# edwinyosorahardjo/compressjs-flattened

Hardware: NVIDIA B200
Metric: bzip2-9 compress MB/s, byte-identical output (higher is better)
Workload: dtype u8

## Files before the change

### compressjs_flattened_b200/csrc/bwt.cuh

```cuda
#pragma once
#include "common.cuh"
#include "rle1.cuh"

#define SORT_TILE 4096
#ifndef SORT_THREADS
#define SORT_THREADS 512
#define SORT_E 8
#endif
#define SEG_THREADS 256
#define SEG_E 16
#define KEEP_BIT 0x80000000u

__global__ void __launch_bounds__(1024) k_tilemap(const u32 *__restrict__ seg_cnt, int nb, u32 *__restrict__ seg_tile0,
                                                  u32 *__restrict__ tile_blk, u64 *__restrict__ totals) {
  __shared__ u32 ws[33];
  __shared__ u64 ws64[33];
  u32 carry = 0;
  u64 act = 0;
  for (int base = 0; base < nb; base += blockDim.x) {
    int p = base + threadIdx.x;
    u32 c = p < nb ? seg_cnt[p] : 0;
    u32 tiles = (c + SORT_TILE - 1) / SORT_TILE, tot;
    u32 t0 = carry + block_excl_sum<u32>(tiles, tot, ws);
    if (p < nb) {
      seg_tile0[p] = t0;
      for (u32 t = 0; t < tiles; t++) tile_blk[t0 + t] = (u32)p;
    }
    carry += tot;
    act += block_sum<u64>((u64)c, ws64);
  }
  if (threadIdx.x == 0) { seg_tile0[nb] = carry; totals[0] = carry; totals[1] = act; }
}

__global__ void k_seg_init(const BlockRec *__restrict__ recs, int nb, u32 *__restrict__ seg_cnt) {
  int p = blockIdx.x * blockDim.x + threadIdx.x;
  if (p < nb) seg_cnt[p] = recs[p].n;
}

struct BlkSort {
  u32 cnt[256];
  u32 L, maxlen;
  u32 pad[6];
  u8 clen[256];
  u16 cval[256];
};
__global__ void __launch_bounds__(256) k_sym_used(const u8 *__restrict__ blk, i64 blk_stride, const BlockRec *__restrict__ recs,
                                                  BlkSort *__restrict__ bs) {
  __shared__ u32 h[8][256];
  const u32 p = blockIdx.y, n = recs[p].n;
  const u8 *T = blk + (i64)p * blk_stride;
  for (int i = threadIdx.x; i < 8 * 256; i += 256) (&h[0][0])[i] = 0;
  __syncthreads();
  u32 *hw = h[warp_id()];
  const u32 nv = n / 16;
  for (u32 x = blockIdx.x * 256 + threadIdx.x; x < nv; x += gridDim.x * 256) {
    uint4 v4 = reinterpret_cast<const uint4 *>(T)[x];
    u32 wv4[4] = {v4.x, v4.y, v4.z, v4.w};
#pragma unroll
    for (int k = 0; k < 16; k++) atomicAdd(&hw[(wv4[k >> 2] >> (8 * (k & 3))) & 0xffu], 1u);
  }
  if (blockIdx.x == 0)
    for (u32 i = nv * 16 + threadIdx.x; i < n; i += 256) atomicAdd(&hw[T[i]], 1u);
  __syncthreads();
  u32 tot = 0;
#pragma unroll
  for (int w = 0; w < 8; w++) tot += h[w][threadIdx.x];
  if (tot) atomicAdd(&bs[p].cnt[threadIdx.x], tot);
}
__global__ void __launch_bounds__(256) k_sym_tab(BlkSort *__restrict__ bs, u32 key_bits, u32 slack) {
  __shared__ u32 ws[33];
  __shared__ u32 P[257];
  __shared__ u32 wmax[8];
  BlkSort &B = bs[blockIdx.x];
  const u32 c = threadIdx.x;
  const u32 f = B.cnt[c];
  u32 used = f ? 1u : 0u, alpha;
  const u32 r = block_excl_sum<u32>(used, alpha, ws);
  u32 tot;
  const u32 pre = block_excl_sum<u32>(f, tot, ws);
  if (used) P[r] = pre;
  if (c == 0) P[alpha] = tot;
  __syncthreads();
  u32 len = 0, val = 0;
  if (used) {
    if (alpha == 1) { len = 1; val = 0; }
    else {
      u32 lb = 1;
      while ((1u << lb) < alpha) lb++;
      const u32 lmax = lb + (alpha > 2 ? slack : 0u);
      u32 lo = 0, hi = alpha;
      while (hi - lo > 1) {
        const u32 cap = 1u << (lmax - len - 1);
        const u64 mid2 = (u64)P[lo] + P[hi];
        u32 a = lo + 1, z = hi - 1;
        while (a < z) {
          const u32 m = (a + z) >> 1;
          if (2ull * P[m] < mid2) a = m + 1; else z = m;
        }
        u32 s = a;
        if (s > lo + 1 && 2ull * P[s] >= mid2 && mid2 - 2ull * P[s - 1] < 2ull * P[s] - mid2) s--;
        const u32 smin = hi > cap + lo ? hi - cap : lo + 1, smax = lo + cap < hi - 1 ? lo + cap : hi - 1;
        if (s < smin) s = smin;
        if (s > smax) s = smax;
        val <<= 1;
        if (r >= s) { val |= 1u; lo = s; } else hi = s;
        len++;
      }
    }
  }
  B.clen[c] = (u8)len;
  B.cval[c] = (u16)val;
  u32 mx = warp_max<u32>(len);
  if (lane_id() == 0) wmax[warp_id()] = mx;
  __syncthreads();
  if (c == 0) {
    u32 m = 1;
    for (int w = 0; w < 8; w++) if (wmax[w] > m) m = wmax[w];
    B.maxlen = m;
    B.L = key_bits / m;
  }
}
__global__ void __launch_bounds__(SEG_THREADS) k_keys_init(const u8 *__restrict__ blk, i64 blk_stride, const BlockRec *__restrict__ recs,
                                                           const u32 *__restrict__ seg_tile0, const u32 *__restrict__ tile_blk,
                                                           const BlkSort *__restrict__ bs, u64 *__restrict__ keys, u32 *__restrict__ hist0,
                                                           u32 tile_base, u32 key_bits) {
  __shared__ u32 cw[256];
  __shared__ u8 sc[SORT_TILE + 48];
  __shared__ u32 h[512];
  __shared__ u64 sk[SORT_TILE];
  u32 tile = blockIdx.x + tile_base, p = tile_blk[tile];
  u32 n = recs[p].n;
  cw[threadIdx.x] = ((u32)bs[p].clen[threadIdx.x] << 16) | bs[p].cval[threadIdx.x];
  for (int i = threadIdx.x; i < 512; i += SEG_THREADS) h[i] = 0;
  __syncthreads();
  const u8 *T = blk + (i64)p * blk_stride;
  u32 l0 = (tile - seg_tile0[p]) * SORT_TILE;
  u64 g0 = (u64)(tile - tile_base) * SORT_TILE;
  const u32 m = n - l0 < SORT_TILE ? n - l0 : SORT_TILE;
  for (u32 j = threadIdx.x; j < m + 43; j += SEG_THREADS) {
    u32 x = l0 + j;
    if (x >= n) x %= n;
    sc[j] = T[x];
  }
  __syncthreads();
  {
    const u32 j0 = threadIdx.x * SEG_E;
    u64 buf = 0;
    u32 bits = 0, kk = j0;
    for (u32 e = 0; e < SEG_E; e++) {
      const u32 j = j0 + e;
      if (j >= m) break;
      while (bits < key_bits) {
        const u32 w = cw[sc[kk++]], l = w >> 16;
        buf |= (u64)(w & 0xffffu) << (64 - bits - l);
        bits += l;
      }
      const u64 key = ((buf >> (64 - key_bits)) << 20) | (l0 + j);
      sk[j] = key;
      atomicAdd(&h[(u32)(key >> 20) & 511u], 1u);
      const u32 lj = cw[sc[j]] >> 16;
      buf <<= lj;
      bits -= lj;
    }
  }
  __syncthreads();
  for (u32 j = threadIdx.x; j < m; j += SEG_THREADS) keys[g0 + j] = sk[j];
  for (int i = threadIdx.x; i < 512; i += SEG_THREADS) hist0[(u64)(tile - tile_base) * 512 + i] = h[i];
}
template <int BITS>
__global__ void __launch_bounds__(SORT_THREADS) k_rs_hist(const u64 *__restrict__ keys, const u32 *__restrict__ seg_cnt,
                                                          const u32 *__restrict__ seg_tile0, const u32 *__restrict__ tile_blk, int shift,
                                                          u32 *__restrict__ hist, const u32 *__restrict__ seg_base, u32 tile_base = 0) {
  constexpr int NB = 1 << BITS;
  __shared__ u32 h[NB];
  u32 tile = blockIdx.x + tile_base, p = tile_blk[tile];
  u32 cnt = seg_cnt[p], l0 = (tile - seg_tile0[p]) * SORT_TILE;
  u64 g0 = seg_base ? (u64)seg_base[p] + l0 : (u64)(tile - tile_base) * SORT_TILE;
  for (int i = threadIdx.x; i < NB; i += SORT_THREADS) h[i] = 0;
  __syncthreads();
  u64 k[SORT_E];
#pragma unroll
  for (int e = 0; e < SORT_E; e++) {
    u32 o = e * SORT_THREADS + threadIdx.x;
    k[e] = l0 + o < cnt ? keys[g0 + o] : 0;
  }
#pragma unroll
  for (int e = 0; e < SORT_E; e++) {
    u32 o = e * SORT_THREADS + threadIdx.x;
    if (l0 + o < cnt) atomicAdd(&h[(u32)(k[e] >> shift) & (NB - 1)], 1u);
  }
  __syncthreads();
  for (int i = threadIdx.x; i < NB; i += SORT_THREADS) hist[(u64)(tile - tile_base) * NB + i] = h[i];
}
#define RSS_WARPS 16
template <int BITS>
__global__ void __launch_bounds__(RSS_WARPS * 32) k_rs_scan(u32 *__restrict__ hist, const u32 *__restrict__ seg_tile0, u32 *__restrict__ digit_tot,
                                                            u32 p_base = 0, u32 tile_base = 0) {
  constexpr int NB = 1 << BITS;
  __shared__ u32 part[RSS_WARPS][32];
  const u32 p = blockIdx.x + p_base, d = blockIdx.y * 32 + lane_id();
  const int w = warp_id();
  const u32 t0 = seg_tile0[p] - tile_base, t1 = seg_tile0[p + 1] - tile_base, nt = t1 - t0;
  const u32 per = (nt + RSS_WARPS - 1) / RSS_WARPS;
  const u32 a = t0 + (u32)w * per < t1 ? t0 + (u32)w * per : t1, b = a + per < t1 ? a + per : t1;
  u32 sum = 0;
  for (u32 t = a; t < b; t++) sum += hist[(u64)t * NB + d];
  part[w][lane_id()] = sum;
  __syncthreads();
  u32 acc = 0;
  for (int ww = 0; ww < w; ww++) acc += part[ww][lane_id()];
  if (w == RSS_WARPS - 1) digit_tot[(u64)p * NB + d] = acc + sum;
  for (u32 t = a; t < b; t++) {
    u32 v = hist[(u64)t * NB + d];
    hist[(u64)t * NB + d] = acc;
    acc += v;
  }
}
template <int BITS>
__global__ void __launch_bounds__(SORT_THREADS, 3) k_rs_scatter(const u64 *__restrict__ keys_in, u64 *__restrict__ keys_out,
                                                             const u32 *__restrict__ seg_cnt, const u32 *__restrict__ seg_tile0,
                                                             const u32 *__restrict__ tile_blk, int shift, const u32 *__restrict__ hist,
                                                             const u32 *__restrict__ digit_tot, const u32 *__restrict__ seg_base, u32 tile_base = 0) {
  constexpr int NB = 1 << BITS;
  __shared__ u16 wcnt[SORT_THREADS / 32][NB];
  __shared__ u32 base[NB];
  u32 tile = blockIdx.x + tile_base, p = tile_blk[tile];
  u32 cnt = seg_cnt[p], l0 = (tile - seg_tile0[p]) * SORT_TILE;
  u64 gp = seg_base ? (u64)seg_base[p] : (u64)(seg_tile0[p] - tile_base) * SORT_TILE, g0 = gp + l0;
  int lane = lane_id(), w = warp_id();
  for (int i = threadIdx.x; i < (SORT_THREADS / 32) * NB / 2; i += SORT_THREADS) reinterpret_cast<u32 *>(&wcnt[0][0])[i] = 0;
  {
    static_assert(NB <= SORT_THREADS, "one digit per thread");
    __shared__ u32 ws[33];
    u32 tot_d = threadIdx.x < NB ? digit_tot[(u64)p * NB + threadIdx.x] : 0u, tot;
    u32 ex = block_excl_sum<u32>(tot_d, tot, ws);
    if (threadIdx.x < NB) base[threadIdx.x] = ex + hist[(u64)(tile - tile_base) * NB + threadIdx.x];
  }
  __syncthreads();
  u64 key[SORT_E];
  u32 rk[SORT_E];
  u32 lt = (1u << lane) - 1;
#pragma unroll
  for (int e = 0; e < SORT_E; e++) {
    u32 o = (u32)w * (32 * SORT_E) + e * 32 + lane;
    key[e] = l0 + o < cnt ? keys_in[g0 + o] : 0;
  }
#pragma unroll
  for (int e = 0; e < SORT_E; e++) {
    u32 o = (u32)w * (32 * SORT_E) + e * 32 + lane;
    bool ok = l0 + o < cnt;
    u32 d = ok ? ((u32)(key[e] >> shift) & (NB - 1)) : (u32)NB;
    u32 peers = __match_any_sync(FULL_MASK, d);
    int leader = __ffs((int)peers) - 1;
    u32 old = 0;
    if (lane == leader && ok) { old = wcnt[w][d]; wcnt[w][d] = (u16)(old + __popc(peers)); }
    old = __shfl_sync(FULL_MASK, old, leader);
    rk[e] = old + __popc(peers & lt);
    __syncwarp();
  }
  __syncthreads();
  for (int d = threadIdx.x; d < NB; d += SORT_THREADS) {
    u32 acc = 0;
    for (int ww = 0; ww < SORT_THREADS / 32; ww++) { u32 t = wcnt[ww][d]; wcnt[ww][d] = (u16)acc; acc += t; }
  }
  __syncthreads();
#pragma unroll
  for (int e = 0; e < SORT_E; e++) {
    u32 o = (u32)w * (32 * SORT_E) + e * 32 + lane;
    if (l0 + o < cnt) {
      u32 d = (u32)(key[e] >> shift) & (NB - 1);
      u64 dst = gp + base[d] + wcnt[w][d] + rk[e];
      keys_out[dst] = key[e];
    }
  }
}

__device__ __forceinline__ void seg_load_flags(const u64 *__restrict__ keys, u64 g0, u32 l0, u32 cnt, int kshift, u64 k[SEG_E], u32 &flags, u32 &lbase) {
  lbase = l0 + threadIdx.x * SEG_E;
  u64 g = g0 + (u64)threadIdx.x * SEG_E;
  flags = 0;
  u64 prev = (lbase > 0 && lbase < cnt) ? keys[g - 1] : 0;
#pragma unroll
  for (int e = 0; e < SEG_E; e++) {
    if (lbase + e < cnt) {
      k[e] = keys[g + e];
      if (lbase + e == 0 || (k[e] >> kshift) != (prev >> kshift)) flags |= 1u << e;
      prev = k[e];
    }
  }
}
__global__ void __launch_bounds__(SEG_THREADS) k_sub_heads(const u64 *__restrict__ keys, const u32 *__restrict__ seg_cnt,
                                                           const u32 *__restrict__ seg_tile0, const u32 *__restrict__ tile_blk,
                                                           int *__restrict__ tile_last, const u32 *__restrict__ seg_base, int kshift) {
  __shared__ int ws[33];
  u32 tile = blockIdx.x, p = tile_blk[tile];
  u32 cnt = seg_cnt[p], l0 = (tile - seg_tile0[p]) * SORT_TILE;
  u64 k[SEG_E];
  u32 flags, lbase;
  seg_load_flags(keys, seg_base ? (u64)seg_base[p] + l0 : (u64)tile * SORT_TILE, l0, cnt, kshift, k, flags, lbase);
  int last = flags ? (int)(lbase + (31 - __clz((int)flags))) : -1;
  last = block_max<int>(last, ws);
  if (threadIdx.x == 0) tile_last[tile] = last;
}
__global__ void __launch_bounds__(256) k_seg_scan(const u32 *__restrict__ seg_tile0, int mode, const int *__restrict__ in, int *__restrict__ out,
                                                  u32 *__restrict__ seg_cnt_new) {
  __shared__ int ws[33];
  u32 p = blockIdx.x, t0 = seg_tile0[p], t1 = seg_tile0[p + 1];
  int carry = mode == 0 ? -1 : 0;
  for (u32 base = t0; base < t1; base += blockDim.x) {
    u32 t = base + threadIdx.x;
    int tot;
    if (mode == 0) {
      int v = t < t1 ? in[t] : -1;
      int e = block_excl_max<int>(v, -1, tot, ws);
      if (t < t1) out[t] = e > carry ? e : carry;
      if (tot > carry) carry = tot;
    } else {
      int v = t < t1 ? in[t] : 0;
      int e = block_excl_sum<int>(v, tot, ws);
      if (t < t1) out[t] = carry + e;
      carry += tot;
    }
  }
  if (mode == 1 && threadIdx.x == 0) seg_cnt_new[p] = (u32)carry;
}
__device__ __forceinline__ void bwt_emit_final(const u8 *__restrict__ T, u8 *__restrict__ L, BlockRec *__restrict__ recs, u32 p, u32 pb, u32 gidx,
                                               u32 rank) {
  if (gidx != pb) L[rank] = T[gidx - 1];
  else {
    L[rank] = T[pb + recs[p].n - 1];
    recs[p].orig_ptr = rank - pb;
  }
}

#define R0_THREADS 512
#define R0_ROWS (SORT_TILE / R0_THREADS)
#define R0_NOKEY 0xffffffffffffffffull
__global__ void __launch_bounds__(R0_THREADS) k_rank0(const u64 *__restrict__ keys, const u32 *__restrict__ seg_cnt,
                                                      const u32 *__restrict__ seg_tile0, const u32 *__restrict__ tile_blk,
                                                      u32 *__restrict__ isa, i64 stride, u32 *__restrict__ act_idx, u32 *__restrict__ act_rank,
                                                      u64 *__restrict__ status, u32 *__restrict__ ticket, u32 *__restrict__ n_act_out, u32 ntiles,
                                                      const u8 *__restrict__ T, u8 *__restrict__ L, BlockRec *__restrict__ recs, u32 tile_base) {
  __shared__ u64 sk[SORT_TILE + 2];
  __shared__ int wlast[R0_THREADS / 32];
  __shared__ u32 wkeep[R0_THREADS / 32];
  __shared__ u32 sh_tile, sh_base;
  __shared__ int sh_carry;
  const int lane = lane_id(), w = warp_id();
  if (threadIdx.x == 0) sh_tile = atomicAdd(ticket, 1u);
  __syncthreads();
  const u32 tile = sh_tile, p = tile_blk[tile];
  const u32 cnt = seg_cnt[p], l0 = (tile - seg_tile0[p]) * SORT_TILE;
  const u64 gp = (u64)(seg_tile0[p] - tile_base) * SORT_TILE;
  const u32 m = cnt - l0 < SORT_TILE ? cnt - l0 : SORT_TILE;
  for (u32 i = threadIdx.x; i < m + 2; i += R0_THREADS) {
    i64 j = (i64)l0 - 1 + i;
    sk[i] = (j >= 0 && j < (i64)cnt) ? keys[gp + (u64)j] : R0_NOKEY;
  }
  __syncthreads();
  u32 hb[R0_ROWS], kb[R0_ROWS];
  int wl = -1;
  u32 nkeep = 0;
#pragma unroll
  for (int e = 0; e < R0_ROWS; e++) {
    u32 i = (u32)w * (32 * R0_ROWS) + e * 32 + lane;
    bool valid = i < m, head = false, nh = false;
    if (valid) {
      u64 k = sk[i + 1] >> 20;
      head = l0 + i == 0 || k != (sk[i] >> 20);
      nh = l0 + i + 1 >= cnt || k != (sk[i + 2] >> 20);
    }
    hb[e] = __ballot_sync(FULL_MASK, head);
    kb[e] = __ballot_sync(FULL_MASK, valid && !(head && nh));
    if (hb[e]) wl = (int)(w * (32 * R0_ROWS) + e * 32 + (31 - __clz((int)hb[e])));
    nkeep += __popc(kb[e]);
  }
  if (lane == 0) { wlast[w] = wl; wkeep[w] = nkeep; }
  if (w == 0) {
    int carry = (int)l0;
    if (l0 > 0 && (sk[1] >> 20) == (sk[0] >> 20)) {
      const u64 P5 = sk[1] >> 20;
      const u64 *K = keys + gp;
      i64 res = -1;
      for (u32 c0 = 0; c0 < 64 && res < 0; c0 += 32) {
        i64 j = (i64)l0 - 2 - c0 - lane;
        bool diff = j < 0 || (K[j] >> 20) != P5;
        u32 b = __ballot_sync(FULL_MASK, diff);
        if (b) res = (i64)l0 - 1 - c0 - (__ffs((int)b) - 1);
      }
      if (res < 0) {
        u32 lo = 0, hi = l0 - 1;
        while (lo < hi) {
          u32 mid = (lo + hi) >> 1;
          if ((K[mid] >> 20) < P5) lo = mid + 1; else hi = mid;
        }
        res = lo;
      }
      carry = (int)res;
    }
    if (lane == 0) sh_carry = carry;
  }
  __syncthreads();
  int cur = sh_carry;
  for (int ww = 0; ww < w; ww++) if (wlast[ww] >= 0) cur = (int)l0 + wlast[ww];
  const u32 pb = (u32)((u64)p * (u64)stride);
  const u32 le = lane == 31 ? 0xffffffffu : ((2u << lane) - 1);
  const u32 lt = (1u << lane) - 1;
  u32 hpv[R0_ROWS];
#pragma unroll
  for (int e = 0; e < R0_ROWS; e++) {
    u32 i = (u32)w * (32 * R0_ROWS) + e * 32 + lane;
    u32 mk = hb[e] & le;
    int hp = mk ? (int)(l0 + w * (32 * R0_ROWS) + e * 32 + (31 - __clz((int)mk))) : cur;
    hpv[e] = (u32)hp;
    if (i < m) {
      const u32 gidx = pb + (u32)(sk[i + 1] & 0xFFFFFu);
      isa[gidx] = (u32)hp;
      if (!((kb[e] >> lane) & 1u)) bwt_emit_final(T, L, recs, p, pb, gidx, pb + (u32)hp);
    }
    if (hb[e]) cur = (int)(l0 + w * (32 * R0_ROWS) + e * 32 + (31 - __clz((int)hb[e])));
  }
  if (w == 0) {
    u32 x = lane < R0_THREADS / 32 ? wkeep[lane] : 0;
    u32 inc = warp_incl_sum<u32>(x);
    u32 agg = __shfl_sync(FULL_MASK, inc, 31);
    u32 base = lookback_warp(status, tile, agg);
    if (lane < R0_THREADS / 32) wkeep[lane] = inc - x;
    if (lane == 0) {
      sh_base = base;
      if (tile == ntiles - 1) *n_act_out = base + agg;
    }
  }
  __syncthreads();
  u32 out = sh_base + wkeep[w];
#pragma unroll
  for (int e = 0; e < R0_ROWS; e++) {
    u32 i = (u32)w * (32 * R0_ROWS) + e * 32 + lane;
    if (i < m && ((kb[e] >> lane) & 1u)) {
      u32 o = out + __popc(kb[e] & lt);
      act_idx[o] = pb + (u32)(sk[i + 1] & 0xFFFFFu);
      act_rank[o] = pb + hpv[e];
    }
    out += __popc(kb[e]);
  }
}
```

### compressjs_flattened_b200/csrc/bz2b200.cu

```cuda
#include "../../include/bz2b200.h"
#include "common.cuh"
#include "rle1.cuh"
#include "bwt.cuh"
#include "refine.cuh"
#include "rsort2.cuh"
#include "mtf.cuh"
#include "huff.cuh"
#include "decode.cuh"

#include <algorithm>
#include <atomic>
#include <chrono>
#include <condition_variable>
#include <future>
#include <mutex>
#include <thread>
#include <cctype>
#include <cstdio>
#include <cstdlib>
#include <fcntl.h>
#include <sched.h>
#include <sys/mman.h>
#include <sys/stat.h>
#include <unistd.h>
#include <string>
#include <utility>
#include <vector>

namespace {

struct ResultPool {
  std::mutex mu;
  std::vector<std::pair<void *, size_t>> live, idle;
  size_t idle_bytes = 0;
  static const size_t kMinPinned = 1 << 20, kMaxIdle = 48;
  static const size_t kMaxIdleBytes = (size_t)12 << 30;
  void *get(size_t bytes) {
    if (bytes < kMinPinned) return malloc(bytes ? bytes : 1);
    std::lock_guard<std::mutex> g(mu);
    size_t best = idle.size();
    for (size_t i = 0; i < idle.size(); i++)
      if (idle[i].second >= bytes && (best == idle.size() || idle[i].second < idle[best].second)) best = i;
    if (best < idle.size()) {
      auto e = idle[best];
      idle.erase(idle.begin() + (long)best);
      idle_bytes -= e.second;
      live.push_back(e);
      return e.first;
    }
    void *p = nullptr;
    size_t cap = bytes + bytes / 4 + 4096;
#ifndef BZ_SIM
    if (cudaMallocHost(&p, cap) != cudaSuccess) { cudaGetLastError(); p = nullptr; }
#endif
    if (!p) return malloc(bytes);
    live.push_back({p, cap});
    return p;
  }
  void put(void *p) {
    if (!p) return;
    {
      std::lock_guard<std::mutex> g(mu);
      for (size_t i = 0; i < live.size(); i++)
        if (live[i].first == p) {
          auto e = live[i];
          live.erase(live.begin() + (long)i);
          if (idle.size() < kMaxIdle && idle_bytes + e.second <= kMaxIdleBytes) { idle.push_back(e); idle_bytes += e.second; return; }
#ifndef BZ_SIM
          cudaFreeHost(p);
#endif
          return;
        }
    }
    free(p);
  }
};
ResultPool &result_pool() { static ResultPool rp; return rp; }

struct DevBuf {
  void *p = nullptr;
  size_t cap = 0;
};

struct Ctx;
struct Pool;
void pool_delete(Pool *p);
struct Ctx {
  Pool *own_pool = nullptr;
  size_t pool_min_bytes = 32000000;
  size_t pool_shard_bytes = 0, pool_halo0 = 0;
  bool pool_force_staging = false;
  int device = 0;
  cudaStream_t stream = nullptr;
  std::string err;
  bz2b200_stats st{};
  std::vector<DevBuf *> pool;
  DevBuf in, tile_last, tile_first, head_carry, tile_emit, g_sub, h_sub, g_tile, recs, nblk, blk, crcpart, pow256;
  DevBuf isa, keysA, keysB, valsB, actI0, actI1, actR0, actR1, lb_status, lbm, hist, digit_base;
  DevBuf seg_cnt, seg_tile0, tile_blk, tile_i0, tile_i1, totals;
  DevBuf Lcol, ranks, lastocc, A, freq, meta, W, bit_off, scrc, out, out_len, used_bits;
  DevBuf rs_tiles, gbounds;
  DevBuf key2, big_cnt, big_old, big_rank, big_tile0, big_tblk, totals2;
  DevBuf recs_cand, cand_first, out2, recs_all, blksort, r2_status, hfreq, hlens, hplen, hcodes, hsel, hcost, hgoff, hblk;
  DevBuf d_in, cand, ncand, dmeta, dsyms, dL, dtt, dwalk, dblk, dout, dmisc, dsel, doff, dperm, dmap;
  struct Pipe {
    const u8 *d_in = nullptr;
    i64 N = 0, T = 0, BS = 0, AS = 0, WS = 0;
    u32 B = 0;
    int level = 9, nb = 0;
    std::vector<BlockRec> hrecs;
  } pipe;
  bool trace = false;
  int sms = 148;
  unsigned ibwt_s = 64;
  u32 r0_tiles = 1u << 30;
  u32 key_slack = 2;
  u32 key_bits = 44;
  bool rs2 = false;
  int parse_mode = 0;
  std::vector<cudaEvent_t> trace_ev, trace_pool;
  std::vector<const char *> trace_names;
  void *rb_pin = nullptr;
  void *rb_dev = nullptr;
  const void *rb_src[4];
  void *rb_dst[4];
  size_t rb_off[4], rb_len[4], rb_used = 0;
  int rb_n = 0;
  u32 rb_seq = 0;
  bool ignore_block_crc = false;
  u32 cap_override = 0;
  u32 batch_override = 0;
  u32 dec_batch = 0;
  u64 shard_bits = 0;
  int cand_n = 0, cand_max_blocks = 0, cand_nb[64];
  i64 cand_s[64];
  bool recs_batched = false;
  int last_nb = 0;
  i64 last_bs = 0, last_as = 0;
  cudaEvent_t ev[10]{};
  bool ev_ok = false;
  std::vector<cudaEvent_t> dom_ev;
  size_t dom_used = 0;
  Ctx() {
    DevBuf *all[] = {&in, &tile_last, &tile_first, &head_carry, &tile_emit, &g_sub, &h_sub, &g_tile, &recs, &nblk, &blk, &crcpart, &pow256,
                     &isa, &keysA, &keysB, &valsB, &actI0, &actI1, &actR0, &actR1, &lb_status, &lbm, &hist, &digit_base,
                     &seg_cnt, &seg_tile0, &tile_blk, &tile_i0, &tile_i1, &totals,
                     &Lcol, &ranks, &lastocc, &A, &freq, &meta, &W, &bit_off, &scrc, &out, &out_len, &used_bits,
                     &rs_tiles, &gbounds, &key2, &big_cnt, &big_old, &big_rank, &big_tile0, &big_tblk, &totals2,
                     &recs_cand, &cand_first, &out2, &recs_all, &blksort, &r2_status, &hfreq, &hlens, &hplen, &hcodes, &hsel, &hcost, &hgoff, &hblk,
                     &d_in, &cand, &ncand, &dmeta, &dsyms, &dL, &dtt, &dwalk, &dblk, &dout, &dmisc, &dsel, &doff, &dperm, &dmap};
    for (DevBuf *b : all) pool.push_back(b);
  }
};

#define CK(call)                                                                         \
  do {                                                                                   \
    cudaError_t _e = (call);                                                             \
    if (_e != cudaSuccess) {                                                             \
      c->err = std::string(#call) + ": " + cudaGetErrorString(_e);                       \
      return BZ2B200_E_CUDA;                                                             \
    }                                                                                    \
  } while (0)

struct RbItem { const void *src; u32 off, bytes; };
__global__ void k_readback(RbItem i0, RbItem i1, RbItem i2, RbItem i3, int n, volatile u8 *host_page, u32 seq) {
  const RbItem it[4] = {i0, i1, i2, i3};
  for (int k = 0; k < n; k++)
    for (u32 b = threadIdx.x; b < it[k].bytes; b += blockDim.x) host_page[it[k].off + b] = reinterpret_cast<const u8 *>(it[k].src)[b];
  __threadfence_system();
  __syncthreads();
  if (threadIdx.x == 0) { *reinterpret_cast<volatile u32 *>(host_page + 1020) = seq; __threadfence_system(); }
}
int rb_add(Ctx *c, void *dst, const void *dev_src, size_t bytes) {
  if (!c->rb_pin) {
#ifndef BZ_SIM
    CK(cudaHostAlloc(&c->rb_pin, 1024, cudaHostAllocMapped));
    CK(cudaHostGetDevicePointer(&c->rb_dev, c->rb_pin, 0));
#else
    CK(cudaMallocHost(&c->rb_pin, 1024));
    c->rb_dev = c->rb_pin;
#endif
    memset(c->rb_pin, 0, 1024);
  }
  if (c->rb_n >= 4 || c->rb_used + bytes > 1000) { c->err = "internal: read-back scratch full"; return BZ2B200_E_CUDA; }
  c->rb_src[c->rb_n] = dev_src;
  c->rb_dst[c->rb_n] = dst; c->rb_off[c->rb_n] = c->rb_used; c->rb_len[c->rb_n] = bytes;
  c->rb_n++;
  c->rb_used += (bytes + 15) & ~(size_t)15;
  return 0;
}
int rb_sync(Ctx *c) {
  if (!c->rb_n) { CK(cudaStreamSynchronize(c->stream)); return 0; }
  RbItem it[4] = {};
  for (int i = 0; i < c->rb_n; i++) { it[i].src = c->rb_src[i]; it[i].off = (u32)c->rb_off[i]; it[i].bytes = (u32)c->rb_len[i]; }
  const u32 seq = ++c->rb_seq;
  KLAUNCH(k_readback, 1, 32, 0, c->stream, it[0], it[1], it[2], it[3], c->rb_n, (volatile u8 *)c->rb_dev, seq);
#ifndef BZ_SIM
  volatile u32 *flag = reinterpret_cast<volatile u32 *>((u8 *)c->rb_pin + 1020);
  for (unsigned spin = 0; *flag != seq; spin++) {
    if ((spin & 0xfffff) == 0xfffff && cudaStreamQuery(c->stream) != cudaErrorNotReady) {
      if (*flag == seq) break;
      CK(cudaStreamSynchronize(c->stream));
      CK(cudaGetLastError());
      c->err = "internal: read-back kernel did not publish";
      return BZ2B200_E_CUDA;
    }
  }
  std::atomic_thread_fence(std::memory_order_acquire);
#endif
  for (int i = 0; i < c->rb_n; i++) memcpy(c->rb_dst[i], (char *)c->rb_pin + c->rb_off[i], c->rb_len[i]);
  c->rb_n = 0;
  c->rb_used = 0;
  return 0;
}
#define RC(call)               \
  do {                         \
    int _r = (call);           \
    if (_r) return _r;         \
  } while (0)

void trace_mark(Ctx *c, const char *name, bool begin) {
#ifndef BZ_SIM
  cudaEvent_t e;
  if (c->trace_pool.size() > c->trace_ev.size()) e = c->trace_pool[c->trace_ev.size()];
  else { if (cudaEventCreate(&e) != cudaSuccess) return; c->trace_pool.push_back(e); }
  cudaEventRecord(e, c->stream);
  c->trace_ev.push_back(e);
  if (begin) c->trace_names.push_back(name);
#else
  (void)c; (void)name; (void)begin;
#endif
}
void trace_report(Ctx *c) {
#ifndef BZ_SIM
  if (!c->trace || c->trace_ev.empty()) return;
  cudaStreamSynchronize(c->stream);
  std::vector<std::pair<std::string, std::pair<int, float>>> agg;
  float gaps = 0, total = 0;
  for (size_t i = 0; i + 1 < c->trace_ev.size(); i += 2) {
    float ms = 0;
    cudaEventElapsedTime(&ms, c->trace_ev[i], c->trace_ev[i + 1]);
    const std::string nm = c->trace_names[i / 2];
    size_t k = 0;
    for (; k < agg.size(); k++) if (agg[k].first == nm) break;
    if (k == agg.size()) agg.push_back({nm, {0, 0.f}});
    agg[k].second.first++;
    agg[k].second.second += ms;
    total += ms;
    if (i + 2 < c->trace_ev.size()) { float g = 0; cudaEventElapsedTime(&g, c->trace_ev[i + 1], c->trace_ev[i + 2]); gaps += g; }
  }
  std::sort(agg.begin(), agg.end(), [](const auto &a, const auto &b) { return a.second.second > b.second.second; });
  fprintf(stderr, "[bz2b200 trace] %zu launches, kernels %.3f ms, gaps between launches %.3f ms\n", c->trace_names.size(), total, gaps);
  for (auto &a : agg) fprintf(stderr, "[bz2b200 trace] %-28s x%-3d %8.3f ms\n", a.first.c_str(), a.second.first, a.second.second);
  c->trace_ev.clear();
  c->trace_names.clear();
#else
  (void)c;
#endif
}

int ensure(Ctx *c, DevBuf &b, size_t bytes) {
  if (bytes <= b.cap) return 0;
  if (b.p) CK(cudaFree(b.p));
  b.p = nullptr;
  b.cap = 0;
  size_t want = bytes + bytes / 8 + 4096;
  CK(cudaMalloc(&b.p, want));
  b.cap = want;
  return 0;
}
#define ENS(buf, bytes)                         \
  do {                                          \
    int _r = ensure(c, (buf), (size_t)(bytes)); \
    if (_r) return _r;                          \
  } while (0)
template <typename T> T *P(DevBuf &b) { return reinterpret_cast<T *>(b.p); }

#define LAUNCH(kern, grid, block, smem, ...)                        \
  do {                                                              \
    if (c->trace) trace_mark(c, #kern, true);                       \
    KLAUNCH(kern, grid, block, smem, c->stream, __VA_ARGS__);       \
    if (c->trace) trace_mark(c, #kern, false);                      \
    c->st.kernel_launches++;                                        \
  } while (0)

inline i64 round_up(i64 v, i64 a) { return (v + a - 1) / a * a; }

int mark(Ctx *c, int i) {
  if (c->ev_ok) CK(cudaEventRecord(c->ev[i], c->stream));
  return 0;
}

int pipe_begin(Ctx *c, const u8 *d_in, size_t n_, int level) {
  if (level < 1 || level > 9) return BZ2B200_E_LEVEL;
  c->st = bz2b200_stats{};
  c->st.in_bytes = n_;
  c->err.clear();
  Ctx::Pipe &P_ = c->pipe;
  P_ = Ctx::Pipe{};
  P_.d_in = d_in; P_.N = (i64)n_; P_.level = level;
  P_.B = c->cap_override ? c->cap_override : (u32)level * 100000u - 19u;
  P_.T = (P_.N + RLE_TILE - 1) / RLE_TILE;
  const i64 N = P_.N, T = P_.T;
  int rc;
  if ((rc = mark(c, 0))) return rc;
  if (N > 0) {
    ENS(c->tile_last, 8 * T); ENS(c->tile_first, 8 * T); ENS(c->head_carry, 8 * T);
    ENS(c->tile_emit, 4 * T); ENS(c->g_tile, 8 * (T + 1));
    LAUNCH(k_rle_heads, (unsigned)T, RLE_THREADS, 0, d_in, N, P<i64>(c->tile_last), P<i64>(c->tile_first));
    LAUNCH(k_scan_excl_max_i64, 1, 1024, 0, P<i64>(c->tile_last), P<i64>(c->head_carry), T);
    ENS(c->g_sub, 4 * (size_t)T * (RLE_THREADS / 32)); ENS(c->h_sub, 8 * (size_t)T * (RLE_THREADS / 32));
    LAUNCH(k_rle_count, (unsigned)T, RLE_THREADS, 0, d_in, N, P<i64>(c->head_carry), P<u32>(c->tile_emit), P<u32>(c->g_sub), P<i64>(c->h_sub));
    LAUNCH(k_scan_excl_sum_u32_u64, 1, 1024, 0, P<u32>(c->tile_emit), P<u64>(c->g_tile), T);
  }
  return BZ2B200_OK;
}

#define CUT_CANDIDATES 64
int pipe_cut(Ctx *c, i64 s_start, i64 own_end, i64 g_start = -1) {
  Ctx::Pipe &P_ = c->pipe;
  const i64 N = P_.N, T = P_.T;
  const u32 B = P_.B;
  const int max_blocks = (int)(N / ((i64)B * 4 / 5) + 2);
  const int ncand = g_start >= 0 ? CUT_CANDIDATES : 1;
  ENS(c->recs, sizeof(BlockRec) * (size_t)max_blocks);
  ENS(c->nblk, 64 + 4 * CUT_CANDIDATES);
  int nb = 0;
  P_.hrecs.clear();
  c->cand_n = 0;
  if (N > 0 && g_start >= 0) {
    ENS(c->recs_cand, sizeof(BlockRec) * (size_t)max_blocks * ncand);
    LAUNCH(k_rle_cut, ncand, CUT_THREADS, 0, P_.d_in, N, B, P<u32>(c->g_sub), P<i64>(c->h_sub), P<i64>(c->tile_first), P<u64>(c->g_tile), T,
           P<BlockRec>(c->recs_cand), max_blocks, P<int>(c->nblk) + 16, s_start, own_end, g_start);
    LAUNCH(k_cand_firsts, 1, CUT_CANDIDATES, 0, P<BlockRec>(c->recs_cand), max_blocks, P<int>(c->nblk) + 16, P<i64>(c->cand_first));
    RC(rb_add(c, c->cand_nb, P<int>(c->nblk) + 16, 4 * CUT_CANDIDATES));
    RC(rb_add(c, c->cand_s, c->cand_first.p, 8 * CUT_CANDIDATES));
    RC(rb_sync(c));
    c->cand_n = ncand;
    c->cand_max_blocks = max_blocks;
  } else if (N > 0 && s_start < N && s_start < own_end) {
    LAUNCH(k_rle_cut, 1, CUT_THREADS, 0, P_.d_in, N, B, P<u32>(c->g_sub), P<i64>(c->h_sub), P<i64>(c->tile_first), P<u64>(c->g_tile), T,
           P<BlockRec>(c->recs), max_blocks, P<int>(c->nblk), s_start, own_end, (i64)-1);
    RC(rb_add(c, &nb, c->nblk.p, sizeof(int)));
    RC(rb_sync(c));
    if (nb < 0) { c->err = "internal: block table overflow"; return BZ2B200_E_CUDA; }
    P_.hrecs.resize((size_t)nb);
    if (nb) CK(cudaMemcpy(P_.hrecs.data(), c->recs.p, sizeof(BlockRec) * (size_t)nb, cudaMemcpyDeviceToHost));
  }
  P_.nb = nb;
  c->st.n_blocks = (u32)nb;
  return BZ2B200_OK;
}
bool pipe_pick(Ctx *c, i64 s_local, i64 own_end, int &rc) {
  Ctx::Pipe &P_ = c->pipe;
  rc = BZ2B200_OK;
  if (!(s_local < P_.N && s_local < own_end)) {
    P_.hrecs.clear();
    P_.nb = 0;
    c->st.n_blocks = 0;
    return true;
  }
  for (int j = 0; j < c->cand_n; j++) {
    const int nbj = c->cand_nb[j];
    if (nbj <= 0 || c->cand_s[j] != s_local) continue;
    P_.hrecs.resize((size_t)nbj);
    const BlockRec *src = P<BlockRec>(c->recs_cand) + (size_t)j * c->cand_max_blocks;
    if (cudaMemcpyAsync(c->recs.p, src, sizeof(BlockRec) * (size_t)nbj, cudaMemcpyDeviceToDevice, c->stream) != cudaSuccess ||
        cudaMemcpy(P_.hrecs.data(), src, sizeof(BlockRec) * (size_t)nbj, cudaMemcpyDeviceToHost) != cudaSuccess) { rc = BZ2B200_E_CUDA; return false; }
    P_.nb = nbj;
    c->st.n_blocks = (u32)nbj;
    return true;
  }
  return false;
}

int pipe_stages(Ctx *c) {
  Ctx::Pipe &P_ = c->pipe;
  const i64 N = P_.N, T = P_.T;
  const u32 B = P_.B;
  const int nb = P_.nb;
  const u8 *d_in = P_.d_in;
  std::vector<BlockRec> &hrecs = P_.hrecs;
  int rc;
  const i64 BS = round_up((i64)B + 1, 256);
  const i64 AS = round_up((i64)B + 2, 128);
  P_.BS = BS; P_.AS = AS;
  c->last_nb = nb; c->last_bs = BS; c->last_as = AS;
  ENS(c->meta, sizeof(BlockMeta) * (size_t)(nb + 1));
  ENS(c->bit_off, 8 * (size_t)(nb + 2));
  ENS(c->scrc, 64);
  ENS(c->out_len, 64);
  i64 WS = 0;
  if (nb) {
    ENS(c->blk, (size_t)nb * BS);
    const i64 t_first = hrecs.front().s / RLE_TILE, t_last = (hrecs.back().p + RLE_TILE - 1) / RLE_TILE;
    (void)T;
    LAUNCH(k_rle_emit, (unsigned)(t_last - t_first), RLE_THREADS, 0, d_in, N, B, P<i64>(c->head_carry), P<u64>(c->g_tile), P<BlockRec>(c->recs), nb,
           P<u8>(c->blk), BS, t_first);
    i64 max_len = 0;
    for (auto &r : hrecs) { if (r.p - r.s > max_len) max_len = r.p - r.s; c->st.rle1_bytes += r.n; }
    int max_chunks = (int)((max_len + CRC_CHUNK - 1) / CRC_CHUNK);
    ENS(c->crcpart, 4 * (size_t)nb * max_chunks);
    if (!c->pow256.p) {
      ENS(c->pow256, 1024);
      u32 h[256];
      for (int j = 0; j < 256; j++) h[j] = crc_xpow(8ull * 256 * (u64)j);
      CK(cudaMemcpy(c->pow256.p, h, sizeof h, cudaMemcpyHostToDevice));
    }
    LAUNCH(k_crc_chunks, dim3((unsigned)max_chunks, (unsigned)nb), 256, 0, d_in, P<BlockRec>(c->recs), P<u32>(c->pow256), P<u32>(c->crcpart),
           max_chunks);
    LAUNCH(k_crc_fold, (unsigned)((nb + 127) / 128), 128, 0, P<BlockRec>(c->recs), nb, P<u32>(c->crcpart), max_chunks,
           crc_xpow(8ull * CRC_CHUNK));
    if ((rc = mark(c, 1))) return rc;

    size_t slots = 0;
    std::vector<u32> tiles_of((size_t)nb), tile_first((size_t)nb);
    for (int b = 0; b < nb; b++) {
      tile_first[(size_t)b] = (u32)(slots / SORT_TILE);
      tiles_of[(size_t)b] = (u32)(round_up(hrecs[(size_t)b].n, SORT_TILE) / SORT_TILE);
      slots += (size_t)tiles_of[(size_t)b] * SORT_TILE;
    }
    const size_t tiles0 = slots / SORT_TILE;
    if ((u64)nb * (u64)BS >= (1ull << 31)) { c->err = "too many bytes for one call (block table * stride must stay below 2^31)"; return BZ2B200_E_ARG; }
    const size_t big_tiles = 5 * tiles0 + 16;
    const u32 big_cap = (u32)(slots / RF_T0 + 16);
    const size_t lb_tiles = slots / RF_T0 + tiles0 + 16;
    ENS(c->isa, 4 * (size_t)nb * BS);
    ENS(c->Lcol, (size_t)nb * BS);
    ENS(c->keysA, 8 * slots); ENS(c->keysB, 8 * slots);
    ENS(c->actI0, 4 * slots); ENS(c->actI1, 4 * slots); ENS(c->actR0, 4 * slots); ENS(c->actR1, 4 * slots);
    ENS(c->key2, 4 * slots);
    ENS(c->hist, 4 * 512 * big_tiles); ENS(c->digit_base, 4 * 512 * (size_t)(big_cap > (u32)nb ? big_cap : (u32)nb));
    ENS(c->seg_cnt, 4 * (size_t)nb); ENS(c->seg_tile0, 4 * (size_t)(nb + 1)); ENS(c->tile_blk, 4 * tiles0);
    ENS(c->tile_i0, 4 * big_tiles); ENS(c->tile_i1, 4 * big_tiles);
    ENS(c->big_cnt, 4 * (size_t)big_cap); ENS(c->big_old, 4 * (size_t)big_cap);
    ENS(c->big_rank, 4 * (size_t)big_cap); ENS(c->big_tile0, 4 * ((size_t)big_cap + 1)); ENS(c->big_tblk, 4 * big_tiles);
    ENS(c->lb_status, 8 * lb_tiles); ENS(c->lbm, 64);
    ENS(c->totals, 64); ENS(c->totals2, 64);
    u32 *seg_cnt = P<u32>(c->seg_cnt), *tile0 = P<u32>(c->seg_tile0), *tblk = P<u32>(c->tile_blk);
    u64 *kA = P<u64>(c->keysA), *kB = P<u64>(c->keysB);
    u32 *actI[2] = {P<u32>(c->actI0), P<u32>(c->actI1)}, *actR[2] = {P<u32>(c->actR0), P<u32>(c->actR1)};
    u32 *lbm = P<u32>(c->lbm);
    u64 *status = P<u64>(c->lb_status);
    const u64 magic = ~0ull / (u64)BS + 1;
    LAUNCH(k_seg_init, (unsigned)((nb + 255) / 256), 256, 0, P<BlockRec>(c->recs), nb, seg_cnt);
    LAUNCH(k_tilemap, 1, 1024, 0, seg_cnt, nb, tile0, tblk, P<u64>(c->totals));
    const unsigned Ta = (unsigned)tiles0;
    ENS(c->blksort, sizeof(BlkSort) * (size_t)nb);
    CK(cudaMemsetAsync(c->blksort.p, 0, sizeof(BlkSort) * (size_t)nb, c->stream));
    LAUNCH(k_sym_used, dim3(32, (unsigned)nb), 256, 0, P<u8>(c->blk), BS, P<BlockRec>(c->recs), P<BlkSort>(c->blksort));
    LAUNCH(k_sym_tab, (unsigned)nb, 256, 0, P<BlkSort>(c->blksort), c->key_bits, c->key_slack);
    ENS(c->rs_tiles, sizeof(RsTile) * (size_t)(Ta + 1));
    if (Ta) LAUNCH(k_rs_tiles, (Ta + 255) / 256, 256, 0, seg_cnt, tile0, tblk, (u32)Ta, P<RsTile>(c->rs_tiles));
    u64 total_n = 0;
    for (auto &r : hrecs) total_n += r.n;
    c->dom_used = 0;
    auto timed_scatter = [&](bool bits9, unsigned grid, const u64 *ki, u64 *ko, const u32 *scnt, const u32 *st0, const u32 *stb, int shift,
                             const u32 *sbase, u64 slots_now, u32 tile_base) -> int {
      if (c->ev_ok) {
        if (c->dom_used + 2 > c->dom_ev.size()) {
          cudaEvent_t a, b2;
          CK(cudaEventCreate(&a)); CK(cudaEventCreate(&b2));
          c->dom_ev.push_back(a); c->dom_ev.push_back(b2);
        }
        CK(cudaEventRecord(c->dom_ev[c->dom_used], c->stream));
      }
      if (bits9) LAUNCH(k_rs_scatter<9>, grid, SORT_THREADS, 0, ki, ko, scnt, st0, stb, shift, P<u32>(c->hist), P<u32>(c->digit_base), sbase, tile_base);
      else LAUNCH(k_rs_scatter<8>, grid, SORT_THREADS, 0, ki, ko, scnt, st0, stb, shift, P<u32>(c->hist), P<u32>(c->digit_base), sbase, tile_base);
      if (c->ev_ok) { CK(cudaEventRecord(c->dom_ev[c->dom_used + 1], c->stream)); c->dom_used += 2; }
      c->st.dom_launches++;
      c->st.dom_bytes += 16ull * slots_now;
      return 0;
    };
    u32 hv[4] = {0, 0, 0, 0};
    {
      c->st.sort_rounds++;
      c->st.sort_slots += (u64)Ta * SORT_TILE;
      CK(cudaMemsetAsync(lbm, 0, 16, c->stream));
      CK(cudaMemsetAsync(status, 0, 8 * (size_t)Ta, c->stream));
      for (int b0 = 0; b0 < nb;) {
        u32 gt = 0;
        int b1 = b0;
        u64 gn = 0;
        while (b1 < nb && (b1 == b0 || gt + tiles_of[b1] <= c->r0_tiles)) { gt += tiles_of[b1]; gn += hrecs[(size_t)b1].n; b1++; }
        const u32 tb = tile_first[b0];
        const unsigned gb = (unsigned)(b1 - b0);
        LAUNCH(k_keys_init, gt, SEG_THREADS, 0, P<u8>(c->blk), BS, P<BlockRec>(c->recs), tile0, tblk, P<BlkSort>(c->blksort), kA, P<u32>(c->hist), tb, c->key_bits);
        u64 *ki = kA, *ko = kB;
        const int npass = (int)(c->key_bits + 8) / 9;
        for (int pass = 0; pass < npass; pass++) {
          if (pass) LAUNCH(k_rs_hist<9>, gt, SORT_THREADS, 0, ki, seg_cnt, tile0, tblk, 20 + pass * 9, P<u32>(c->hist), (const u32 *)nullptr, tb);
          if (c->rs2 && tb == 0 && gt == Ta) {
#if RS2_SCAN1
            LAUNCH(k_rs_scan<9>, dim3((unsigned)nb, 512 / 32), RSS_WARPS * 32, 0, P<u32>(c->hist), tile0, P<u32>(c->digit_base), 0u, 0u);
#else
            LAUNCH(k_rs_bases, (unsigned)nb, 512, 0, P<u32>(c->hist), tile0);
#endif
            if (c->ev_ok) {
              if (c->dom_used + 2 > c->dom_ev.size()) {
                cudaEvent_t a, b2;
                CK(cudaEventCreate(&a)); CK(cudaEventCreate(&b2));
                c->dom_ev.push_back(a); c->dom_ev.push_back(b2);
              }
              CK(cudaEventRecord(c->dom_ev[c->dom_used], c->stream));
            }
            const unsigned g2 = gt < (unsigned)(2 * c->sms) ? gt : (unsigned)(2 * c->sms);
            LAUNCH(k_rs_scatter2, g2, RS2_THREADS, sizeof(Rs2Smem), ki, ko, P<u32>(c->hist), P<RsTile>(c->rs_tiles), gt, 20 + pass * 9, P<u32>(c->digit_base));
            if (c->ev_ok) { CK(cudaEventRecord(c->dom_ev[c->dom_used + 1], c->stream)); c->dom_used += 2; }
            c->st.dom_launches++;
            c->st.dom_bytes += 16ull * gn;
          } else {
            LAUNCH(k_rs_scan<9>, dim3(gb, 512 / 32), RSS_WARPS * 32, 0, P<u32>(c->hist), tile0, P<u32>(c->digit_base), (u32)b0, tb);
            if ((rc = timed_scatter(true, gt, ki, ko, seg_cnt, tile0, tblk, 20 + pass * 9, nullptr, gn, tb))) return rc;
          }
          u64 *tk = ki; ki = ko; ko = tk;
        }
        LAUNCH(k_rank0, gt, R0_THREADS, 0, ki, seg_cnt, tile0, tblk, P<u32>(c->isa), BS, actI[0], actR[0], status, lbm, lbm + 1, (u32)Ta, P<u8>(c->blk),
               P<u8>(c->Lcol), P<BlockRec>(c->recs), tb);
        b0 = b1;
      }
      RC(rb_add(c, hv, lbm, sizeof hv));
      RC(rb_sync(c));
    }
    u32 n_act = hv[1], round = 0;
    if (n_act) LAUNCH(k_keys2, (n_act + 255) / 256, 256, 0, actI[0], n_act, P<BlockRec>(c->recs), P<u32>(c->isa), (u32)BS, magic, P<BlkSort>(c->blksort), round,
                      P<u32>(c->key2));
    while (n_act) {
      c->st.sort_rounds++;
      c->st.sort_slots += n_act;
      const u32 ntiles = (n_act + RF_T0 - 1) / RF_T0, ctiles = (n_act + CK_TILE - 1) / CK_TILE;
      CK(cudaMemsetAsync(lbm, 0, 16, c->stream));
      CK(cudaMemsetAsync(status, 0, 8 * (size_t)ctiles, c->stream));
      ENS(c->gbounds, 8 * ((size_t)ntiles + 2));
      u32 *gb_lo = P<u32>(c->gbounds), *gb_lo2 = gb_lo + ntiles + 1;
      LAUNCH(k_group_bounds, (ntiles + 1 + 7) / 8, 256, 0, actR[0], n_act, ntiles, gb_lo, gb_lo2, P<u32>(c->big_cnt), P<u32>(c->big_old), P<u32>(c->big_rank),
             lbm + 2, big_cap);
      LAUNCH(k_sort_groups, ntiles, RF_THREADS, sizeof(RfSmem), P<u32>(c->key2), actI[0], actR[0], n_act, P<u32>(c->isa), (u32)BS, magic, actI[1],
             actR[1], P<u32>(c->big_cnt), P<u32>(c->big_old), P<u32>(c->big_rank), lbm + 2, big_cap, P<u8>(c->blk), P<u8>(c->Lcol), P<BlockRec>(c->recs),
             gb_lo, gb_lo2);
      RC(rb_add(c, hv, lbm, sizeof hv));
      RC(rb_sync(c));
      const u32 n_big = hv[2];
      if (n_big > big_cap) { c->err = "internal: big-group list overflow"; return BZ2B200_E_CUDA; }
      if (n_big) {
        u32 *bcnt = P<u32>(c->big_cnt), *bbase = P<u32>(c->big_old), *bt0 = P<u32>(c->big_tile0), *btb = P<u32>(c->big_tblk);
        u64 t2[2] = {0, 0};
        LAUNCH(k_tilemap, 1, 1024, 0, bcnt, (int)n_big, bt0, btb, P<u64>(c->totals2));
        RC(rb_add(c, t2, c->totals2.p, sizeof t2));
        RC(rb_sync(c));
        const unsigned Tb = (unsigned)t2[0];
        LAUNCH(k_big_keys, Tb, SEG_THREADS, 0, P<u32>(c->key2), actI[0], bcnt, bt0, btb, bbase, kA);
        u64 *ki = kA, *ko = kB;
        for (int pass = 0; pass < 3; pass++) {
          LAUNCH(k_rs_hist<8>, Tb, SORT_THREADS, 0, ki, bcnt, bt0, btb, 32 + pass * 8, P<u32>(c->hist), bbase);
          LAUNCH(k_rs_scan<8>, dim3(n_big, 256 / 32), RSS_WARPS * 32, 0, P<u32>(c->hist), bt0, P<u32>(c->digit_base));
          if ((rc = timed_scatter(false, Tb, ki, ko, bcnt, bt0, btb, 32 + pass * 8, bbase, t2[1], 0u))) return rc;
          u64 *tk = ki; ki = ko; ko = tk;
        }
        LAUNCH(k_sub_heads, Tb, SEG_THREADS, 0, ki, bcnt, bt0, btb, P<int>(c->tile_i0), bbase, 32);
        LAUNCH(k_seg_scan, n_big, 256, 0, bt0, 0, P<int>(c->tile_i0), P<int>(c->tile_i1), (u32 *)nullptr);
        LAUNCH(k_big_apply, Tb, SEG_THREADS, 0, ki, bcnt, bt0, btb, bbase, P<u32>(c->big_rank), P<int>(c->tile_i1), P<u32>(c->isa), (u32)BS, magic,
               actI[1], actR[1], P<u8>(c->blk), P<u8>(c->Lcol), P<BlockRec>(c->recs));
      }
      round = round < 30 ? round + 1 : round;
      LAUNCH(k_compact_keys, ctiles, CK_THREADS, 0, actI[1], actR[1], n_act, P<BlockRec>(c->recs), P<u32>(c->isa), (u32)BS, magic, P<BlkSort>(c->blksort), round,
             actI[0], actR[0],
             P<u32>(c->key2), status, lbm, lbm + 1, ctiles);
      RC(rb_add(c, hv, lbm, sizeof hv));
      RC(rb_sync(c));
      n_act = hv[1];
    }
    if ((rc = mark(c, 2))) return rc;

    const i64 nseg_max = (BS + MTF_SEG - 1) / MTF_SEG;
    ENS(c->ranks, (size_t)nb * BS);
    ENS(c->lastocc, 4 * 256 * (size_t)nseg_max * nb);
    ENS(c->A, 2 * (size_t)nb * AS);
    ENS(c->freq, 4 * BZ_MAX_SYMS * (size_t)nb);
    ENS(c->used_bits, 32 * (size_t)nb);
    CK(cudaMemsetAsync(c->used_bits.p, 0, 32 * (size_t)nb, c->stream));
    LAUNCH(k_mtf_lastocc, dim3((unsigned)((nseg_max + 7) / 8), (unsigned)nb), 256, 0, P<u8>(c->Lcol), BS, P<BlockRec>(c->recs), P<int>(c->lastocc),
           nseg_max * 256, P<u32>(c->used_bits));
    LAUNCH(k_mtf_scan, (unsigned)nb, 256, 0, P<BlockRec>(c->recs), P<int>(c->lastocc), nseg_max * 256, P<u32>(c->used_bits), P<BlockMeta>(c->meta));
    LAUNCH(k_mtf_ranks, dim3((unsigned)((nseg_max + MTR_WARPS - 1) / MTR_WARPS), (unsigned)nb), MTR_WARPS * 32, MTR_WARPS * sizeof(MtrSmem), P<u8>(c->Lcol),
           BS, P<BlockRec>(c->recs), P<int>(c->lastocc), nseg_max * 256, P<u8>(c->ranks));
    {
      const i64 r2_tiles = (BS + R2_TILE - 1) / R2_TILE;
      ENS(c->r2_status, 8 * (size_t)nb * r2_tiles + 4 * (size_t)nb);
      CK(cudaMemsetAsync(c->r2_status.p, 0, 8 * (size_t)nb * r2_tiles + 4 * (size_t)nb, c->stream));
      CK(cudaMemsetAsync(c->freq.p, 0, 4 * BZ_MAX_SYMS * (size_t)nb, c->stream));
      LAUNCH(k_mtf_rle2, dim3((unsigned)r2_tiles, (unsigned)nb), R2_THREADS, 0, P<BlockRec>(c->recs), P<u8>(c->ranks), BS, P<u16>(c->A), AS, P<u32>(c->freq),
             P<BlockMeta>(c->meta), P<u64>(c->r2_status), r2_tiles, reinterpret_cast<u32 *>(P<u64>(c->r2_status) + (size_t)nb * r2_tiles));
    }
    if ((rc = mark(c, 3))) return rc;

    u64 maxbits = 80 + 25 + 16 + 256 + 18 + 7ull * ((B + 1 + 49) / 50) + 6ull * (5 + 258 * 39) + 20ull * (B + 1);
    WS = round_up((i64)((maxbits + 31) / 32) + 2, 64);
    ENS(c->W, 4 * (size_t)nb * WS);
    const u32 max_nsel = (B + 1 + BZ_GROUP - 1) / BZ_GROUP;
    HufArrays ha;
    ha.sel_stride = round_up((i64)max_nsel + 1, 16);
    ENS(c->hfreq, 4 * (size_t)nb * BZ_MAX_GROUPS * BZ_MAX_SYMS);
    ENS(c->hlens, (size_t)nb * BZ_MAX_GROUPS * HUF_LSTRIDE);
    ENS(c->hplen, 8 * (size_t)nb * BZ_MAX_SYMS);
    ENS(c->hcodes, 4 * (size_t)nb * BZ_MAX_GROUPS * BZ_MAX_SYMS);
    ENS(c->hsel, (size_t)nb * ha.sel_stride);
    ENS(c->hcost, 2 * (size_t)nb * ha.sel_stride);
    ENS(c->hgoff, 4 * (size_t)nb * ha.sel_stride);
    ENS(c->hblk, sizeof(HufBlk) * (size_t)nb);
    ha.freq = P<u32>(c->hfreq); ha.lens = P<u8>(c->hlens); ha.plen = P<u64>(c->hplen); ha.codes = P<u32>(c->hcodes);
    ha.sel = P<u8>(c->hsel); ha.cost = P<u16>(c->hcost); ha.goff = P<u32>(c->hgoff); ha.hb = P<HufBlk>(c->hblk);
    const dim3 ggrid((max_nsel + HUF_GT - 1) / HUF_GT, (unsigned)nb);
    LAUNCH(k_huf_init, (unsigned)nb, HUF_BT, sizeof(HufBuildSmem), ha, P<u32>(c->freq), P<BlockMeta>(c->meta));
    for (int it = 0; it < BZ_MAX_GROUPS - 2; it++) {
      LAUNCH(k_huf_assign, ggrid, HUF_GT, 0, ha, P<u16>(c->A), AS, 0);
      LAUNCH(k_huf_split, (unsigned)nb, HUF_BT, 0, ha);
      LAUNCH(k_huf_hist, ggrid, HUF_GT, 0, ha, P<u16>(c->A), AS);
      LAUNCH(k_huf_build, (unsigned)nb, HUF_BT, sizeof(HufBuildSmem), ha);
    }
    LAUNCH(k_huf_assign, ggrid, HUF_GT, 0, ha, P<u16>(c->A), AS, 1);
    LAUNCH(k_huf_codes, (unsigned)nb, HUF_CT, 0, ha, P<BlockRec>(c->recs), P<BlockMeta>(c->meta), P<u32>(c->W), WS);
    LAUNCH(k_huf_emit, ggrid, HUF_GT, 0, ha, P<u16>(c->A), AS, P<u32>(c->W), WS);
  } else {
    for (int i = 1; i <= 3; i++) if ((rc = mark(c, i))) return rc;
  }
  P_.WS = WS;
  if ((rc = mark(c, 4))) return rc;
  return BZ2B200_OK;
}

int pipe_emit(Ctx *c, u64 base_bits, bool whole, u32 *d_out, size_t out_cap, bool own_out, size_t *out_len, u64 *bits_out, u32 *crc_fold) {
  Ctx::Pipe &P_ = c->pipe;
  const int nb = P_.nb;
  LAUNCH(k_stitch_offsets, 1, 1024, 0, P<BlockMeta>(c->meta), P<BlockRec>(c->recs), nb, P<u64>(c->bit_off), P<u32>(c->scrc), base_bits);
  u64 end_bits = 0;
  u32 fold = 0;
  RC(rb_add(c, &end_bits, P<u64>(c->bit_off) + nb, 8));
  RC(rb_add(c, &fold, c->scrc.p, 4));
  RC(rb_sync(c));
  if (bits_out) *bits_out = end_bits - base_bits;
  if (crc_fold) *crc_fold = fold;
  size_t need = (size_t)((end_bits + (whole ? 80 : 0) + 7) / 8);
  size_t need_w = round_up((i64)need, 4) + 8;
  if (own_out) {
    ENS(c->out, need_w);
    d_out = P<u32>(c->out);
  } else if (out_cap < need_w) {
    c->err = "output buffer too small";
    return BZ2B200_E_UNEXPECTED_OUTPUT_EOF;
  }
  CK(cudaMemsetAsync(d_out, 0, need_w, c->stream));
  if (nb) LAUNCH(k_stitch, dim3(32, (unsigned)nb), 256, 0, P<u32>(c->W), P_.WS, P<u64>(c->bit_off), d_out);
  u64 olen = need;
  if (whole) {
    LAUNCH(k_stream_ends, 1, 32, 0, d_out, P<u64>(c->bit_off), nb, P<u32>(c->scrc), P_.level, P<u64>(c->out_len));
    RC(rb_add(c, &olen, c->out_len.p, 8));
  }
  int rc;
  if ((rc = mark(c, 5))) return rc;
  RC(rb_sync(c));
  CK(cudaGetLastError());
  *out_len = (size_t)olen;
  c->st.out_bytes = olen;
  if (nb) {
    std::vector<BlockMeta> hm((size_t)nb);
    CK(cudaMemcpy(hm.data(), c->meta.p, sizeof(BlockMeta) * (size_t)nb, cudaMemcpyDeviceToHost));
    c->st.mtf_syms = 0;
    for (auto &m : hm) { c->st.mtf_syms += m.m; c->st.d1_triggered |= m.d1; }
  }
  if (c->ev_ok) {
    for (int i = 0; i < 5; i++) CK(cudaEventElapsedTime(&c->st.ms_stage[i], c->ev[i], c->ev[i + 1]));
    CK(cudaEventElapsedTime(&c->st.ms_total, c->ev[0], c->ev[5]));
    c->st.dom_ms = 0;
    for (size_t i = 0; i + 1 < c->dom_used; i += 2) {
      float ms = 0;
      CK(cudaEventElapsedTime(&ms, c->dom_ev[i], c->dom_ev[i + 1]));
      c->st.dom_ms += ms;
    }
  }
  return BZ2B200_OK;
}

int batch_limit(Ctx *c) {
  if (c->batch_override) return (int)c->batch_override;
  const i64 BS = round_up((i64)c->pipe.B + 1, 256);
  const i64 by_index = ((1ll << 31) - 1) / BS;
  i64 by_mem = by_index;
#ifndef BZ_SIM
  size_t pooled = 0;
  for (DevBuf *b : c->pool) pooled += b->cap;
  const size_t need = (size_t)c->pipe.nb * (size_t)BS * 52;
  if (need > pooled) {
    size_t free_b = 0, total_b = 0;
    if (cudaMemGetInfo(&free_b, &total_b) == cudaSuccess) by_mem = (i64)((free_b + pooled) / 10 * 7 / (size_t)(BS * 52));
  }
#endif
  i64 lim = by_index < by_mem ? by_index : by_mem;
  return (int)(lim < 1 ? 1 : lim);
}

int pipe_emit_part(Ctx *c, u64 base_bits, bool first, u32 *d_out, size_t out_cap, u64 *bits_out, u32 *crc_fold) {
  Ctx::Pipe &P_ = c->pipe;
  const int nb = P_.nb;
  LAUNCH(k_stitch_offsets, 1, 1024, 0, P<BlockMeta>(c->meta), P<BlockRec>(c->recs), nb, P<u64>(c->bit_off), P<u32>(c->scrc), base_bits);
  u64 end_bits = 0;
  u32 fold = 0;
  RC(rb_add(c, &end_bits, P<u64>(c->bit_off) + nb, 8));
  RC(rb_add(c, &fold, c->scrc.p, 4));
  RC(rb_sync(c));
  *bits_out = end_bits - base_bits;
  *crc_fold = fold;
  const u64 w_first = first ? 0 : (base_bits >> 5) + 1, w_end = ((end_bits + 80 + 31) >> 5) + 2;
  if (w_end * 4 > out_cap) { c->err = "output buffer too small"; return BZ2B200_E_UNEXPECTED_OUTPUT_EOF; }
  if (w_end > w_first) CK(cudaMemsetAsync(d_out + w_first, 0, (size_t)(w_end - w_first) * 4, c->stream));
  if (nb) LAUNCH(k_stitch, dim3(32, (unsigned)nb), 256, 0, P<u32>(c->W), P_.WS, P<u64>(c->bit_off), d_out);
  int rc;
  if ((rc = mark(c, 5))) return rc;
  CK(cudaStreamSynchronize(c->stream));
  CK(cudaGetLastError());
  return BZ2B200_OK;
}

int pipe_run(Ctx *c, u64 base_bits, bool whole, u32 *d_out, size_t out_cap, bool own_out, size_t *out_len, u64 *bits_out, u32 *crc_fold) {
  Ctx::Pipe &P_ = c->pipe;
  const int nb_total = P_.nb, maxb = batch_limit(c);
  int rc;
  c->recs_batched = false;
  if (nb_total <= maxb) {
    if ((rc = pipe_stages(c))) return rc;
    return pipe_emit(c, base_bits, whole, d_out, out_cap, own_out, out_len, bits_out, crc_fold);
  }
  std::vector<BlockRec> all = P_.hrecs;
  ENS(c->recs_all, sizeof(BlockRec) * (size_t)nb_total);
  CK(cudaMemcpyAsync(c->recs_all.p, c->recs.p, sizeof(BlockRec) * (size_t)nb_total, cudaMemcpyDeviceToDevice, c->stream));
  if (own_out) {
    out_cap = bz2b200_compress_bound((size_t)P_.N, P_.level) + 64;
    ENS(c->out, out_cap);
    d_out = P<u32>(c->out);
  }
  u64 running = base_bits, mtf_syms = 0;
  u32 fold = 0, d1 = 0;
  float ms_stage[5] = {0, 0, 0, 0, 0}, ms_total = 0, dom_ms = 0;
  for (int b0 = 0; b0 < nb_total; b0 += maxb) {
    const int bn = nb_total - b0 < maxb ? nb_total - b0 : maxb;
    CK(cudaMemcpyAsync(c->recs.p, P<BlockRec>(c->recs_all) + b0, sizeof(BlockRec) * (size_t)bn, cudaMemcpyDeviceToDevice, c->stream));
    P_.hrecs.assign(all.begin() + b0, all.begin() + b0 + bn);
    P_.nb = bn;
    if (b0) { if ((rc = mark(c, 0))) return rc; if ((rc = mark(c, 1))) return rc; }
    if ((rc = pipe_stages(c))) return rc;
    u64 bits = 0;
    u32 foldb = 0;
    if ((rc = pipe_emit_part(c, running, b0 == 0, d_out, out_cap, &bits, &foldb))) return rc;
    CK(cudaMemcpyAsync(P<BlockRec>(c->recs_all) + b0, c->recs.p, sizeof(BlockRec) * (size_t)bn, cudaMemcpyDeviceToDevice, c->stream));
    const u32 m = (u32)bn & 31u;
    fold = (m ? ((fold << m) | (fold >> (32 - m))) : fold) ^ foldb;
    running += bits;
    {
      std::vector<BlockMeta> hm((size_t)bn);
      CK(cudaMemcpy(hm.data(), c->meta.p, sizeof(BlockMeta) * (size_t)bn, cudaMemcpyDeviceToHost));
      for (auto &mm : hm) { mtf_syms += mm.m; d1 |= mm.d1; }
    }
    if (c->ev_ok) {
      for (int i = 0; i < 5; i++) { float t = 0; CK(cudaEventElapsedTime(&t, c->ev[i], c->ev[i + 1])); ms_stage[i] += t; ms_total += t; }
      for (size_t i = 0; i + 1 < c->dom_used; i += 2) { float t = 0; CK(cudaEventElapsedTime(&t, c->dom_ev[i], c->dom_ev[i + 1])); dom_ms += t; }
    }
  }
  P_.hrecs = all;
  P_.nb = nb_total;
  c->recs_batched = true;
  c->st.n_blocks = (u32)nb_total;
  if (bits_out) *bits_out = running - base_bits;
  if (crc_fold) *crc_fold = fold;
  u64 olen = (running + 7) / 8;
  if (whole) {
    u64 endb = running;
    CK(cudaMemcpyAsync(c->bit_off.p, &endb, 8, cudaMemcpyHostToDevice, c->stream));
    CK(cudaMemcpyAsync(c->scrc.p, &fold, 4, cudaMemcpyHostToDevice, c->stream));
    LAUNCH(k_stream_ends, 1, 32, 0, d_out, P<u64>(c->bit_off), 0, P<u32>(c->scrc), P_.level, P<u64>(c->out_len));
    RC(rb_add(c, &olen, c->out_len.p, 8));
    RC(rb_sync(c));
  }
  *out_len = (size_t)olen;
  c->st.out_bytes = olen;
  c->st.mtf_syms = mtf_syms;
  c->st.d1_triggered = d1;
  for (int i = 0; i < 5; i++) c->st.ms_stage[i] = ms_stage[i];
  c->st.ms_total = ms_total;
  c->st.dom_ms = dom_ms;
  return BZ2B200_OK;
}

int compress_device(Ctx *c, const u8 *d_in, size_t n_, int level, u32 *d_out, size_t out_cap, size_t *out_len, bool own_out) {
  int rc;
  if ((rc = pipe_begin(c, d_in, n_, level))) return rc;
  if ((rc = pipe_cut(c, 0, (i64)n_))) return rc;
  rc = pipe_run(c, 32, true, d_out, out_cap, own_out, out_len, nullptr, nullptr);
  trace_report(c);
  return rc;
}

#include "decode_host.inl"
#include "pool.inl"

cudaError_t set_kernel_attributes() {
#ifndef BZ_SIM
  cudaError_t e;
  if ((e = cudaFuncSetAttribute(k_sort_groups, cudaFuncAttributeMaxDynamicSharedMemorySize, (int)sizeof(RfSmem))) != cudaSuccess) return e;
  if ((e = cudaFuncSetAttribute(k_rs_scatter2, cudaFuncAttributeMaxDynamicSharedMemorySize, (int)sizeof(Rs2Smem))) != cudaSuccess) return e;
  if ((e = cudaFuncSetAttribute(k_mtf_ranks, cudaFuncAttributeMaxDynamicSharedMemorySize, (int)(MTR_WARPS * sizeof(MtrSmem)))) != cudaSuccess) return e;
  if ((e = cudaFuncSetAttribute(k_huf_init, cudaFuncAttributeMaxDynamicSharedMemorySize, (int)sizeof(HufBuildSmem))) != cudaSuccess) return e;
  if ((e = cudaFuncSetAttribute(k_huf_build, cudaFuncAttributeMaxDynamicSharedMemorySize, (int)sizeof(HufBuildSmem))) != cudaSuccess) return e;
  if ((e = cudaFuncSetAttribute(k_huff_parse_win, cudaFuncAttributeMaxDynamicSharedMemorySize, (int)sizeof(DecWinSmem))) != cudaSuccess) return e;
  const size_t rank_smem = 12 * (size_t)((DEC_DBUF_MAX + 64 - 1) / 64 + 2);
  if ((e = cudaFuncSetAttribute(k_ibwt_rank, cudaFuncAttributeMaxDynamicSharedMemorySize, (int)rank_smem)) != cudaSuccess) return e;
#endif
  return cudaSuccess;
}

int ctx_new(int device, Ctx **out) {
  int ndev = 0;
  if (cudaGetDeviceCount(&ndev) != cudaSuccess || ndev <= 0 || device < 0 || device >= ndev) return BZ2B200_E_CUDA;
  if (cudaSetDevice(device) != cudaSuccess) return BZ2B200_E_CUDA;
  Ctx *c = new Ctx();
  c->device = device;
  if (cudaStreamCreate(&c->stream) != cudaSuccess) { delete c; return BZ2B200_E_CUDA; }
  c->ev_ok = true;
  { const char *t = getenv("BZ2B200_TRACE"); c->trace = t && *t && *t != '0'; }
  { const char *t = getenv("BZ2B200_PARSE"); c->parse_mode = t ? atoi(t) : 0; }
  { const char *t = getenv("BZ2B200_KEY_SLACK"); if (t && *t >= '0' && *t <= '3') c->key_slack = (u32)(*t - '0'); }
  { const char *t = getenv("BZ2B200_KEY_BITS"); int v = t ? atoi(t) : 0; if (v == 36 || v == 44 || v == 27) c->key_bits = (u32)v; }
  { const char *t = getenv("BZ2B200_RS2"); if (t && *t) c->rs2 = *t != '0'; }
  { const char *t = getenv("BZ2B200_R0_TILES"); int v = t ? atoi(t) : 0; if (v > 0) c->r0_tiles = (u32)v; }
  { const char *t = getenv("BZ2B200_IBWT_S"); int v = t ? atoi(t) : 0; if (v == 64 || v == 128 || v == 256 || v == 512 || v == 1024) c->ibwt_s = (unsigned)v; }
  { int v = 0; if (cudaDeviceGetAttribute(&v, cudaDevAttrMultiProcessorCount, device) == cudaSuccess && v > 0) c->sms = v; }
  for (auto &e : c->ev) if (cudaEventCreate(&e) != cudaSuccess) c->ev_ok = false;
  if (set_kernel_attributes() != cudaSuccess) { ctx_delete(c); return BZ2B200_E_CUDA; }
  *out = c;
  return BZ2B200_OK;
}

void ctx_delete(Ctx *c) {
  if (!c) return;
  if (c->own_pool) pool_delete(c->own_pool);
  cudaSetDevice(c->device);
  for (DevBuf *b : c->pool) if (b->p) cudaFree(b->p);
  if (c->rb_pin) cudaFreeHost(c->rb_pin);
  for (auto &e : c->ev) if (e) cudaEventDestroy(e);
  for (auto &e : c->dom_ev) cudaEventDestroy(e);
  for (auto &e : c->trace_pool) cudaEventDestroy(e);
  cudaStreamDestroy(c->stream);
  delete c;
}

}

extern "C" {

int bz2b200_create(int device, bz2b200_ctx **ctx) {
  if (!ctx) return BZ2B200_E_ARG;
  *ctx = nullptr;
  Ctx *c = nullptr;
  int rc = ctx_new(device, &c);
  if (rc) return rc;
  *ctx = reinterpret_cast<bz2b200_ctx *>(c);
  return BZ2B200_OK;
}

void bz2b200_destroy(bz2b200_ctx *ctx) { ctx_delete(reinterpret_cast<Ctx *>(ctx)); }

int bz2b200_compress_device(bz2b200_ctx *ctx, const void *d_in, size_t n, int level, void *d_out, size_t out_cap, size_t *out_len) {
  Ctx *c = reinterpret_cast<Ctx *>(ctx);
  if (!c || !out_len || (n && !d_in) || !d_out || ((uintptr_t)d_in & 15) || ((uintptr_t)d_out & 3)) return BZ2B200_E_ARG;
  CK(cudaSetDevice(c->device));
  return compress_device(c, (const u8 *)d_in, n, level, (u32 *)d_out, out_cap, out_len, false);
}

int bz2b200_compress(bz2b200_ctx *ctx, const uint8_t *in, size_t n, int level, uint8_t **out, size_t *out_len) {
  Ctx *c = reinterpret_cast<Ctx *>(ctx);
  if (!c || !out || !out_len || (n && !in)) return BZ2B200_E_ARG;
  if (level < 1 || level > 9) return BZ2B200_E_LEVEL;
  CK(cudaSetDevice(c->device));
  if (n >= c->pool_min_bytes) {
    if (!c->own_pool) {
      const int dev = c->device;
      int prc = pool_new(&dev, 1, 2, &c->own_pool);
      if (prc) { c->err = "cannot create the lanes of the context's pool"; return prc; }
    }
    Pool *p = c->own_pool;
    p->cap_override = c->cap_override; p->batch_override = c->batch_override;
    p->halo0 = c->pool_halo0; p->force_staging = c->pool_force_staging;
    p->plan_first = n / 5 * 2 + 1;
    p->plan_growth = 1000.0;
    int prc = pool_compress_whole(p, in, n, level, c->pool_shard_bytes, out, out_len);
    c->st = p->st;
    c->err = p->err;
    return prc;
  }
  ENS(c->in, n + 64);
  if (n) CK(cudaMemcpyAsync(c->in.p, in, n, cudaMemcpyHostToDevice, c->stream));
  size_t olen = 0;
  int rc = compress_device(c, P<u8>(c->in), n, level, nullptr, 0, &olen, true);
  if (rc) return rc;
  uint8_t *res = (uint8_t *)result_pool().get(olen);
  if (!res) return BZ2B200_E_OUT_OF_MEMORY;
  CK(cudaMemcpy(res, c->out.p, olen, cudaMemcpyDeviceToHost));
  *out = res;
  *out_len = olen;
  return BZ2B200_OK;
}

int bz2b200_shard_begin(bz2b200_ctx *ctx, const void *in, size_t n_avail, int on_device, int level) {
  Ctx *c = reinterpret_cast<Ctx *>(ctx);
  if (!c || (n_avail && !in)) return BZ2B200_E_ARG;
  if (level < 1 || level > 9) return BZ2B200_E_LEVEL;
  CK(cudaSetDevice(c->device));
  const u8 *d_in = (const u8 *)in;
  if (!on_device) {
    ENS(c->in, n_avail + 64);
    if (n_avail) CK(cudaMemcpyAsync(c->in.p, in, n_avail, cudaMemcpyHostToDevice, c->stream));
    d_in = P<u8>(c->in);
  } else if ((uintptr_t)in & 15) return BZ2B200_E_ARG;
  return pipe_begin(c, d_in, n_avail, level);
}

static void shard_fill_info(Ctx *c, i64 s_start, int is_last, bz2b200_shard_info *info) {
  *info = bz2b200_shard_info{};
  const auto &h = c->pipe.hrecs;
  info->n_blocks = (uint32_t)h.size();
  info->next_start = h.empty() ? (uint64_t)(s_start < 0 ? 0 : s_start) : (uint64_t)h.back().p;
  info->complete = 1;
  if (!is_last && !h.empty() && h.back().p == c->pipe.N && h.back().n < c->pipe.B) info->complete = 0;
}

int bz2b200_shard_cut(bz2b200_ctx *ctx, uint64_t s_start, uint64_t own_len, int is_last, bz2b200_shard_info *info) {
  Ctx *c = reinterpret_cast<Ctx *>(ctx);
  if (!c || !info) return BZ2B200_E_ARG;
  CK(cudaSetDevice(c->device));
  if ((i64)own_len > c->pipe.N) own_len = (uint64_t)c->pipe.N;
  int rc = pipe_cut(c, (i64)s_start, (i64)own_len);
  if (rc) return rc;
  shard_fill_info(c, (i64)s_start, is_last, info);
  return BZ2B200_OK;
}

int bz2b200_shard_gtotal(bz2b200_ctx *ctx, uint64_t pos, uint64_t *g) {
  Ctx *c = reinterpret_cast<Ctx *>(ctx);
  if (!c || !g) return BZ2B200_E_ARG;
  CK(cudaSetDevice(c->device));
  const i64 N = c->pipe.N;
  *g = 0;
  if (N == 0) return BZ2B200_OK;
  ENS(c->nblk, 64 + 4 * CUT_CANDIDATES);
  LAUNCH(k_rle_gquery, 1, 32, 0, c->pipe.d_in, N, P<u32>(c->g_sub), P<i64>(c->h_sub), P<u64>(c->g_tile), c->pipe.T, (i64)(pos > (uint64_t)N ? (uint64_t)N : pos),
         P<u64>(c->nblk) + 1);
  u64 v = 0;
  RC(rb_add(c, &v, P<u64>(c->nblk) + 1, 8));
  RC(rb_sync(c));
  *g = v;
  return BZ2B200_OK;
}

int bz2b200_shard_cut_g(bz2b200_ctx *ctx, uint64_t g_before, uint64_t own_len) {
  Ctx *c = reinterpret_cast<Ctx *>(ctx);
  if (!c) return BZ2B200_E_ARG;
  CK(cudaSetDevice(c->device));
  c->cand_n = 0;
  if (c->pipe.N == 0) return BZ2B200_OK;
  if ((i64)own_len > c->pipe.N) own_len = (uint64_t)c->pipe.N;
  const u64 B = c->pipe.B, g_start = (B - g_before % B) % B;
  ENS(c->cand_first, 8 * CUT_CANDIDATES);
  return pipe_cut(c, 0, (i64)own_len, (i64)g_start);
}

int bz2b200_shard_cut_pick(bz2b200_ctx *ctx, uint64_t s_start, uint64_t own_len, int is_last, bz2b200_shard_info *info, int *found) {
  Ctx *c = reinterpret_cast<Ctx *>(ctx);
  if (!c || !info || !found) return BZ2B200_E_ARG;
  CK(cudaSetDevice(c->device));
  if ((i64)own_len > c->pipe.N) own_len = (uint64_t)c->pipe.N;
  int rc = BZ2B200_OK;
  *found = pipe_pick(c, (i64)s_start, (i64)own_len, rc) ? 1 : 0;
  if (rc) return rc;
  if (*found) shard_fill_info(c, (i64)s_start, is_last, info);
  return BZ2B200_OK;
}

int bz2b200_shard_compress(bz2b200_ctx *ctx, bz2b200_shard_info *info) {
  Ctx *c = reinterpret_cast<Ctx *>(ctx);
  if (!c || !info) return BZ2B200_E_ARG;
  CK(cudaSetDevice(c->device));
  size_t olen = 0;
  u64 bits = 0;
  u32 fold = 0;
  int rc = pipe_run(c, 0, false, nullptr, 0, true, &olen, &bits, &fold);
  if (rc) return rc;
  c->shard_bits = bits;
  info->bits = bits;
  info->crc_fold = fold;
  return BZ2B200_OK;
}

int bz2b200_shard_emit(bz2b200_ctx *ctx, int bit_phase, bz2b200_shard_info *info, uint8_t **seg, size_t *seg_bytes) {
  Ctx *c = reinterpret_cast<Ctx *>(ctx);
  if (!c || !info || !seg_bytes || bit_phase < 0 || bit_phase > 7) return BZ2B200_E_ARG;
  CK(cudaSetDevice(c->device));
  const u64 bits = c->shard_bits, nsrc = (bits + 7) / 8;
  const size_t olen = (size_t)(((u64)bit_phase + bits + 7) / 8);
  const u8 *d_seg = P<u8>(c->out);
  if (bit_phase && bits) {
    ENS(c->out2, nsrc + 16);
    LAUNCH(k_shift_bytes, (unsigned)((nsrc + 256) / 256), 256, 0, P<u8>(c->out), nsrc, (u32)bit_phase, P<u8>(c->out2));
    d_seg = P<u8>(c->out2);
  }
  CK(cudaStreamSynchronize(c->stream));
  info->bit_phase = (uint32_t)bit_phase;
  *seg_bytes = olen;
  if (!seg) return BZ2B200_OK;
  uint8_t *res = (uint8_t *)result_pool().get(olen);
  if (!res) return BZ2B200_E_OUT_OF_MEMORY;
  if (olen) CK(cudaMemcpy(res, d_seg, olen, cudaMemcpyDeviceToHost));
  *seg = res;
  *seg_bytes = olen;
  return BZ2B200_OK;
}

int bz2b200_stitch_shards(int level, int n_shards, const uint8_t *const *segs, const bz2b200_shard_info *infos, uint8_t **out, size_t *out_len) {
  if (level < 1 || level > 9) return BZ2B200_E_LEVEL;
  if (n_shards < 0 || !out || !out_len || (n_shards && (!segs || !infos))) return BZ2B200_E_ARG;
  u64 total_bits = 32;
  for (int r = 0; r < n_shards; r++) total_bits += infos[r].bits;
  size_t nbytes = (size_t)((total_bits + 80 + 7) / 8);
  uint8_t *o = (uint8_t *)calloc(nbytes + 8, 1);
  if (!o) return BZ2B200_E_OUT_OF_MEMORY;
  o[0] = 'B'; o[1] = 'Z'; o[2] = 'h'; o[3] = (uint8_t)('0' + level);
  u64 bitpos = 32;
  u32 crc = 0;
  for (int r = 0; r < n_shards; r++) {
    if (infos[r].bits) {
      if (infos[r].bit_phase != (u32)(bitpos & 7)) { free(o); return BZ2B200_E_ARG; }
      size_t off = (size_t)(bitpos >> 3), len = (size_t)((infos[r].bit_phase + infos[r].bits + 7) / 8);
      o[off] |= segs[r][0];
      if (len > 1) memcpy(o + off + 1, segs[r] + 1, len - 1);
      bitpos += infos[r].bits;
    }
    u32 m = infos[r].n_blocks & 31u;
    crc = (m ? ((crc << m) | (crc >> (32 - m))) : crc) ^ infos[r].crc_fold;
  }
  u64 vals[2] = {BZ_MAGIC_END, (u64)crc};
  int lens[2] = {48, 32};
  for (int q = 0; q < 2; q++)
    for (int i = lens[q] - 1; i >= 0; i--, bitpos++)
      if ((vals[q] >> i) & 1) o[bitpos >> 3] |= (uint8_t)(0x80u >> (bitpos & 7));
  *out = o;
  *out_len = (size_t)((bitpos + 7) / 8);
  return BZ2B200_OK;
}

size_t bz2b200_compress_bound(size_t n, int level) {
  if (level < 1 || level > 9) level = 9;
  size_t B = (size_t)level * 100000 - 19;
  size_t nblocks = n / (B * 4 / 5) + 2;
  return (n + n / 4 + nblocks) / 8 * 9 + nblocks * 22000 + 1024;
}

void bz2b200_free(void *p) { result_pool().put(p); }

const char *bz2b200_strerror(int rc) {
  switch (rc) {
    case BZ2B200_OK: return "OK";
    case BZ2B200_E_LAST_BLOCK: return "Bad file checksum";
    case BZ2B200_E_NOT_BZIP_DATA: return "Not bzip data";
    case BZ2B200_E_UNEXPECTED_INPUT_EOF: return "Unexpected input EOF";
    case BZ2B200_E_UNEXPECTED_OUTPUT_EOF: return "Unexpected output EOF";
    case BZ2B200_E_DATA_ERROR: return "Data error";
    case BZ2B200_E_OUT_OF_MEMORY: return "Out of memory";
    case BZ2B200_E_OBSOLETE_INPUT: return "Obsolete (pre 0.9.5) bzip format not supported.";
    case BZ2B200_E_LEVEL: return "Invalid block size multiplier";
    case BZ2B200_E_CUDA: return "CUDA failure";
    case BZ2B200_E_ARG: return "bad argument";
    case BZ2B200_E_PEER: return "a peer of the shard group failed or timed out";
    default: return "unknown error";
  }
}

const char *bz2b200_last_error(bz2b200_ctx *ctx) {
  Ctx *c = reinterpret_cast<Ctx *>(ctx);
  return c ? c->err.c_str() : "no context";
}

int bz2b200_last_stats(bz2b200_ctx *ctx, bz2b200_stats *st) {
  Ctx *c = reinterpret_cast<Ctx *>(ctx);
  if (!c || !st) return BZ2B200_E_ARG;
  *st = c->st;
  return BZ2B200_OK;
}

long long bz2b200_debug_fetch(bz2b200_ctx *ctx, int what, int blk, void *dst, size_t cap) {
  Ctx *c = reinterpret_cast<Ctx *>(ctx);
  if (!c || !dst) return BZ2B200_E_ARG;
  const void *src = nullptr;
  size_t bytes = 0;
  int nb = c->last_nb;
  if (what != 0 && what != 4 && (blk < 0 || blk >= nb)) return BZ2B200_E_ARG;
  switch (what) {
    case 0:
      if (c->recs_batched) { src = c->recs_all.p; bytes = sizeof(BlockRec) * (size_t)c->pipe.nb; }
      else { src = c->recs.p; bytes = sizeof(BlockRec) * (size_t)nb; }
      break;
    case 1: src = P<u8>(c->blk) + (i64)blk * c->last_bs; bytes = (size_t)c->last_bs; break;
    case 2: src = P<u8>(c->Lcol) + (i64)blk * c->last_bs; bytes = (size_t)c->last_bs; break;
    case 3: src = P<u16>(c->A) + (i64)blk * c->last_as; bytes = 2 * (size_t)c->last_as; break;
    case 4: src = c->meta.p; bytes = sizeof(BlockMeta) * (size_t)nb; break;
    default: return BZ2B200_E_ARG;
  }
  if (bytes > cap) bytes = cap;
  if (bytes && cudaMemcpy(dst, src, bytes, cudaMemcpyDeviceToHost) != cudaSuccess) return BZ2B200_E_CUDA;
  return (long long)bytes;
}

int bz2b200_debug_huffman_lengths(bz2b200_ctx *ctx, int32_t *a, int n, int maxlen) {
  Ctx *c = reinterpret_cast<Ctx *>(ctx);
  if (!c || !a || n < 0 || n > 1 << 20 || maxlen < 1 || maxlen > 32) return BZ2B200_E_ARG;
  CK(cudaSetDevice(c->device));
  if (!n) return BZ2B200_OK;
  ENS(c->dmisc, 4 * (size_t)n + 64);
  CK(cudaMemcpyAsync(c->dmisc.p, a, 4 * (size_t)n, cudaMemcpyHostToDevice, c->stream));
  LAUNCH(k_debug_ha_allocate, 1, 32, 0, P<int>(c->dmisc), n, maxlen);
  CK(cudaMemcpyAsync(a, c->dmisc.p, 4 * (size_t)n, cudaMemcpyDeviceToHost, c->stream));
  CK(cudaStreamSynchronize(c->stream));
  return BZ2B200_OK;
}

int bz2b200_debug_set_batch_blocks(bz2b200_ctx *ctx, uint32_t blocks) {
  Ctx *c = reinterpret_cast<Ctx *>(ctx);
  if (!c) return BZ2B200_E_ARG;
  c->batch_override = blocks;
  return BZ2B200_OK;
}

int bz2b200_debug_set_ignore_block_crc(bz2b200_ctx *ctx, int on) {
  Ctx *c = reinterpret_cast<Ctx *>(ctx);
  if (!c) return BZ2B200_E_ARG;
  c->ignore_block_crc = on != 0;
  return BZ2B200_OK;
}

int bz2b200_debug_set_block_cap(bz2b200_ctx *ctx, uint32_t cap) {
  Ctx *c = reinterpret_cast<Ctx *>(ctx);
  if (!c || (cap && cap < 8) || cap > 899981) return BZ2B200_E_ARG;
  c->cap_override = cap;
  return BZ2B200_OK;
}

#include "decode_abi.inl"
#include "pool_abi.inl"
#include "stream_abi.inl"

}
```

### compressjs_flattened_b200/csrc/rsort2.cuh

```cuda
#pragma once
#include "common.cuh"
#include "bwt.cuh"

struct RsTile {
  u32 p;
  u32 m;
  u32 g0;
  u32 gp;
};
__global__ void k_rs_tiles(const u32 *__restrict__ seg_cnt, const u32 *__restrict__ seg_tile0, const u32 *__restrict__ tile_blk, u32 ntiles,
                           RsTile *__restrict__ info) {
  u32 t = blockIdx.x * blockDim.x + threadIdx.x;
  if (t >= ntiles) return;
  u32 p = tile_blk[t], l0 = (t - seg_tile0[p]) * SORT_TILE, cnt = seg_cnt[p];
  RsTile r;
  r.p = p; r.m = cnt - l0 < SORT_TILE ? cnt - l0 : SORT_TILE; r.g0 = t * SORT_TILE; r.gp = seg_tile0[p] * SORT_TILE;
  info[t] = r;
}

__global__ void __launch_bounds__(512) k_rs_bases(u32 *__restrict__ hist, const u32 *__restrict__ seg_tile0) {
  __shared__ u32 ws[33];
  const u32 p = blockIdx.x, d = threadIdx.x;
  const u32 t0 = seg_tile0[p], t1 = seg_tile0[p + 1];
  u32 sum = 0;
  for (u32 t = t0; t < t1; t++) sum += hist[(u64)t * 512 + d];
  u32 tot;
  u32 acc = block_excl_sum<u32>(sum, tot, ws);
  for (u32 t = t0; t < t1; t++) {
    const u32 v = hist[(u64)t * 512 + d];
    hist[(u64)t * 512 + d] = acc;
    acc += v;
  }
}

#ifndef RS2_BALLOT
#define RS2_BALLOT 0
#endif
#ifndef RS2_PACK
#define RS2_PACK 1
#endif
#ifndef RS2_SCAN1
#define RS2_SCAN1 1
#endif
#ifndef RS2_DIRECT
#define RS2_DIRECT 0
#endif
#define RS2_THREADS 512
#define RS2_WARPS (RS2_THREADS / 32)
struct Rs2Smem {
  u64 keys[2][SORT_TILE];
  u32 gbase[2][512];
#if RS2_SCAN1
  u32 dtot[2][512];
#endif
#if RS2_PACK
  u32 wcnt[RS2_WARPS / 2][512];
#else
  u32 wcnt[RS2_WARPS][512];
#endif
  u32 lpos[512];
  u32 delta[512];
  u32 ws[34];
  u64 ws64[34];
  RsTile info[2];
  u64 mbar[2];
};

#ifndef BZ_SIM
__device__ __forceinline__ u32 smem_u32(const void *p) { return (u32)__cvta_generic_to_shared(p); }
__device__ __forceinline__ void mbar_init(u64 *bar, u32 count) { asm volatile("mbarrier.init.shared::cta.b64 [%0], %1;" ::"r"(smem_u32(bar)), "r"(count)); }
__device__ __forceinline__ void mbar_expect_tx(u64 *bar, u32 bytes) {
  asm volatile("mbarrier.arrive.expect_tx.shared::cta.b64 _, [%0], %1;" ::"r"(smem_u32(bar)), "r"(bytes) : "memory");
}
__device__ __forceinline__ void tma_load_1d(void *dst, const void *src, u32 bytes, u64 *bar) {
  asm volatile("cp.async.bulk.shared::cluster.global.mbarrier::complete_tx::bytes [%0], [%1], %2, [%3];" ::"r"(smem_u32(dst)), "l"(src), "r"(bytes),
               "r"(smem_u32(bar))
               : "memory");
}
__device__ __forceinline__ void mbar_wait(u64 *bar, u32 parity) {
  asm volatile(
      "{\n"
      ".reg .pred p;\n"
      "RS2_WAIT:\n"
      "mbarrier.try_wait.parity.shared::cta.b64 p, [%0], %1;\n"
      "@p bra RS2_DONE;\n"
      "bra RS2_WAIT;\n"
      "RS2_DONE:\n"
      "}\n" ::"r"(smem_u32(bar)),
      "r"(parity)
      : "memory");
}
#endif

__device__ __forceinline__ void rs2_fetch(Rs2Smem &sm, int b, u32 tile, const u64 *__restrict__ keys_in, const u32 *__restrict__ hist,
                                          const RsTile *__restrict__ tinfo, const u32 *__restrict__ digit_tot) {
  const RsTile ti = tinfo[tile];
  sm.info[b] = ti;
  const u32 kbytes = ((ti.m * 8u) + 15u) & ~15u;
#ifndef BZ_SIM
  asm volatile("fence.proxy.async.shared::cta;" ::: "memory");
  mbar_expect_tx(&sm.mbar[b], kbytes + 2048u * (1 + RS2_SCAN1));
  tma_load_1d(sm.keys[b], keys_in + ti.g0, kbytes, &sm.mbar[b]);
  tma_load_1d(sm.gbase[b], hist + (u64)tile * 512, 2048u, &sm.mbar[b]);
#if RS2_SCAN1
  tma_load_1d(sm.dtot[b], digit_tot + (u64)ti.p * 512, 2048u, &sm.mbar[b]);
#endif
#else
  for (u32 i = 0; i < kbytes / 8; i++) sm.keys[b][i] = keys_in[ti.g0 + i];
  for (u32 i = 0; i < 512; i++) sm.gbase[b][i] = hist[(u64)tile * 512 + i];
#if RS2_SCAN1
  for (u32 i = 0; i < 512; i++) sm.dtot[b][i] = digit_tot[(u64)ti.p * 512 + i];
#endif
#endif
  (void)digit_tot;
}

__global__ void __launch_bounds__(RS2_THREADS, 2) k_rs_scatter2(const u64 *__restrict__ keys_in, u64 *__restrict__ keys_out, const u32 *__restrict__ hist,
                                                                const RsTile *__restrict__ tinfo, u32 ntiles, int shift,
                                                                const u32 *__restrict__ digit_tot) {
  DYN_SMEM(Rs2Smem, smp);
  Rs2Smem &sm = *smp;
  const int lane = lane_id(), w = warp_id();
  const u32 lt = (1u << lane) - 1;
  if (threadIdx.x == 0) {
#ifndef BZ_SIM
    mbar_init(&sm.mbar[0], 1);
    mbar_init(&sm.mbar[1], 1);
    asm volatile("fence.mbarrier_init.release.cluster;" ::: "memory");
#endif
  }
  __syncthreads();
  u32 tile = blockIdx.x;
  if (threadIdx.x == 0 && tile < ntiles) rs2_fetch(sm, 0, tile, keys_in, hist, tinfo, digit_tot);
  for (u32 it = 0; tile < ntiles; it++, tile += gridDim.x) {
    const int b = (int)(it & 1);
    if (threadIdx.x == 0 && tile + gridDim.x < ntiles) rs2_fetch(sm, b ^ 1, tile + gridDim.x, keys_in, hist, tinfo, digit_tot);
#ifndef BZ_SIM
    mbar_wait(&sm.mbar[b], (it >> 1) & 1u);
#else
    __syncthreads();
#endif
    const u32 m = sm.info[b].m, gp = sm.info[b].gp;
    u64 key[SORT_E];
    u32 rk[SORT_E];
#pragma unroll
    for (int e = 0; e < SORT_E; e++) {
      const u32 o = (u32)w * (32 * SORT_E) + e * 32 + lane;
      key[e] = o < m ? sm.keys[b][o] : 0;
    }
#if RS2_PACK
    for (int i = threadIdx.x; i < RS2_WARPS / 2 * 512; i += RS2_THREADS) (&sm.wcnt[0][0])[i] = 0;
#else
    for (int i = threadIdx.x; i < RS2_WARPS * 512; i += RS2_THREADS) (&sm.wcnt[0][0])[i] = 0;
#endif
    u32 dg[SORT_E], peers[SORT_E];
#pragma unroll
    for (int e = 0; e < SORT_E; e++) {
      const u32 o = (u32)w * (32 * SORT_E) + e * 32 + lane;
      dg[e] = o < m ? ((u32)(key[e] >> shift) & 511u) : 512u;
#if RS2_BALLOT
      u32 pm = __ballot_sync(FULL_MASK, o < m);
      if (!(o < m)) pm = ~pm;
#pragma unroll
      for (int bit = 0; bit < 9; bit++) {
        const bool one = (dg[e] >> bit) & 1u;
        const u32 bal = __ballot_sync(FULL_MASK, one);
        pm &= one ? bal : ~bal;
      }
      peers[e] = pm;
#else
      peers[e] = __match_any_sync(FULL_MASK, dg[e]);
#endif
    }
    __syncthreads();
#pragma unroll
    for (int e = 0; e < SORT_E; e++) {
      const int leader = __ffs((int)peers[e]) - 1;
      u32 old = 0;
#if RS2_PACK
      if (lane == leader && dg[e] < 512u) old = (atomicAdd(&sm.wcnt[w >> 1][dg[e]], (u32)__popc(peers[e]) << (16 * (w & 1))) >> (16 * (w & 1))) & 0xffffu;
#else
      if (lane == leader && dg[e] < 512u) old = atomicAdd(&sm.wcnt[w][dg[e]], (u32)__popc(peers[e]));
#endif
      old = __shfl_sync(FULL_MASK, old, leader);
      rk[e] = old + __popc(peers[e] & lt);
    }
    __syncthreads();
    {
      const u32 d = threadIdx.x;
      u32 acc = 0;
#if RS2_PACK
      u32 cw[RS2_WARPS / 2];
#pragma unroll
      for (int q = 0; q < RS2_WARPS / 2; q++) {
        const u32 v = sm.wcnt[q][d], lo = v & 0xffffu, hi = v >> 16;
        cw[q] = acc | ((acc + lo) << 16);
        acc += lo + hi;
      }
#if RS2_SCAN1
      u64 tot64;
      const u64 ex = block_excl_sum<u64>(((u64)sm.dtot[b][d] << 32) | acc, tot64, reinterpret_cast<u64 *>(sm.ws64));
      const u32 lp = (u32)ex, dbase = (u32)(ex >> 32);
#else
      u32 tot;
      const u32 lp = block_excl_sum<u32>(acc, tot, sm.ws);
      const u32 dbase = 0;
#endif
#pragma unroll
      for (int q = 0; q < RS2_WARPS / 2; q++) sm.wcnt[q][d] = cw[q] + lp * 0x10001u;
#else
      u32 cw[RS2_WARPS];
#pragma unroll
      for (int ww = 0; ww < RS2_WARPS; ww++) { cw[ww] = acc; acc += sm.wcnt[ww][d]; }
      u32 tot;
      const u32 lp = block_excl_sum<u32>(acc, tot, sm.ws);
      const u32 dbase = 0;
#pragma unroll
      for (int ww = 0; ww < RS2_WARPS; ww++) sm.wcnt[ww][d] = lp + cw[ww];
#endif
      sm.lpos[d] = lp;
      sm.delta[d] = dbase + sm.gbase[b][d] - lp;
    }
    __syncthreads();
#if RS2_DIRECT
#pragma unroll
    for (int e = 0; e < SORT_E; e++)
      if (dg[e] < 512u) {
#if RS2_PACK
        const u32 slot = ((sm.wcnt[w >> 1][dg[e]] >> (16 * (w & 1))) & 0xffffu) + rk[e];
#else
        const u32 slot = sm.wcnt[w][dg[e]] + rk[e];
#endif
        keys_out[(u64)gp + sm.delta[dg[e]] + slot] = key[e];
      }
#else
#pragma unroll
    for (int e = 0; e < SORT_E; e++)
      if (dg[e] < 512u) {
#if RS2_PACK
        sm.keys[b][((sm.wcnt[w >> 1][dg[e]] >> (16 * (w & 1))) & 0xffffu) + rk[e]] = key[e];
#else
        sm.keys[b][sm.wcnt[w][dg[e]] + rk[e]] = key[e];
#endif
      }
    __syncthreads();
    for (u32 i = threadIdx.x; i < m; i += RS2_THREADS) {
      const u64 k = sm.keys[b][i];
      keys_out[(u64)gp + sm.delta[(u32)(k >> shift) & 511u] + i] = k;
    }
#endif
    __syncthreads();
  }
}
```

Baseline: 7449.

## Replace tiled radix passes with per-bucket merge sort for small digit buckets

Removes the TMA-pipelined rs_scatter2 path and the tile_base chunking. It adds a planning kernel that groups small digit buckets (at most 4096 keys) into work items and finishes each item with a shared-memory bitonic-network-plus-merge-path sort. Only oversized buckets are forwarded to further radix passes. The aim is to skip full-array radix passes for keys already separated by the top digit, at the cost of device atomics for item allocation and padded shared-memory merge passes.

```diff
diff --git a/compressjs_flattened_b200/csrc/bwt.cuh b/compressjs_flattened_b200/csrc/bwt.cuh
--- a/compressjs_flattened_b200/csrc/bwt.cuh
+++ b/compressjs_flattened_b200/csrc/bwt.cuh
@@ -12,9 +12,10 @@
 #define KEEP_BIT 0x80000000u
 
 __global__ void __launch_bounds__(1024) k_tilemap(const u32 *__restrict__ seg_cnt, int nb, u32 *__restrict__ seg_tile0,
-                                                  u32 *__restrict__ tile_blk, u64 *__restrict__ totals) {
+                                                  u32 *__restrict__ tile_blk, u64 *__restrict__ totals, const u32 *__restrict__ nb_dev = nullptr) {
   __shared__ u32 ws[33];
   __shared__ u64 ws64[33];
+  if (nb_dev) nb = (int)*nb_dev;
   u32 carry = 0;
   u64 act = 0;
   for (int base = 0; base < nb; base += blockDim.x) {
@@ -123,19 +124,19 @@
 __global__ void __launch_bounds__(SEG_THREADS) k_keys_init(const u8 *__restrict__ blk, i64 blk_stride, const BlockRec *__restrict__ recs,
                                                            const u32 *__restrict__ seg_tile0, const u32 *__restrict__ tile_blk,
                                                            const BlkSort *__restrict__ bs, u64 *__restrict__ keys, u32 *__restrict__ hist0,
-                                                           u32 tile_base, u32 key_bits) {
+                                                           u32 hshift, u32 key_bits) {
   __shared__ u32 cw[256];
   __shared__ u8 sc[SORT_TILE + 48];
   __shared__ u32 h[512];
   __shared__ u64 sk[SORT_TILE];
-  u32 tile = blockIdx.x + tile_base, p = tile_blk[tile];
+  u32 tile = blockIdx.x, p = tile_blk[tile];
   u32 n = recs[p].n;
   cw[threadIdx.x] = ((u32)bs[p].clen[threadIdx.x] << 16) | bs[p].cval[threadIdx.x];
   for (int i = threadIdx.x; i < 512; i += SEG_THREADS) h[i] = 0;
   __syncthreads();
   const u8 *T = blk + (i64)p * blk_stride;
   u32 l0 = (tile - seg_tile0[p]) * SORT_TILE;
-  u64 g0 = (u64)(tile - tile_base) * SORT_TILE;
+  u64 g0 = (u64)tile * SORT_TILE;
   const u32 m = n - l0 < SORT_TILE ? n - l0 : SORT_TILE;
   for (u32 j = threadIdx.x; j < m + 43; j += SEG_THREADS) {
     u32 x = l0 + j;
@@ -157,7 +158,7 @@
       }
       const u64 key = ((buf >> (64 - key_bits)) << 20) | (l0 + j);
       sk[j] = key;
-      atomicAdd(&h[(u32)(key >> 20) & 511u], 1u);
+      atomicAdd(&h[(u32)(key >> hshift) & 511u], 1u);
       const u32 lj = cw[sc[j]] >> 16;
       buf <<= lj;
       bits -= lj;
@@ -165,17 +166,17 @@
   }
   __syncthreads();
   for (u32 j = threadIdx.x; j < m; j += SEG_THREADS) keys[g0 + j] = sk[j];
-  for (int i = threadIdx.x; i < 512; i += SEG_THREADS) hist0[(u64)(tile - tile_base) * 512 + i] = h[i];
+  for (int i = threadIdx.x; i < 512; i += SEG_THREADS) hist0[(u64)tile * 512 + i] = h[i];
 }
 template <int BITS>
 __global__ void __launch_bounds__(SORT_THREADS) k_rs_hist(const u64 *__restrict__ keys, const u32 *__restrict__ seg_cnt,
                                                           const u32 *__restrict__ seg_tile0, const u32 *__restrict__ tile_blk, int shift,
-                                                          u32 *__restrict__ hist, const u32 *__restrict__ seg_base, u32 tile_base = 0) {
+                                                          u32 *__restrict__ hist, const u32 *__restrict__ seg_base) {
   constexpr int NB = 1 << BITS;
   __shared__ u32 h[NB];
-  u32 tile = blockIdx.x + tile_base, p = tile_blk[tile];
+  u32 tile = blockIdx.x, p = tile_blk[tile];
   u32 cnt = seg_cnt[p], l0 = (tile - seg_tile0[p]) * SORT_TILE;
-  u64 g0 = seg_base ? (u64)seg_base[p] + l0 : (u64)(tile - tile_base) * SORT_TILE;
+  u64 g0 = seg_base ? (u64)seg_base[p] + l0 : (u64)tile * SORT_TILE;
   for (int i = threadIdx.x; i < NB; i += SORT_THREADS) h[i] = 0;
   __syncthreads();
   u64 k[SORT_E];
@@ -190,17 +191,16 @@
     if (l0 + o < cnt) atomicAdd(&h[(u32)(k[e] >> shift) & (NB - 1)], 1u);
   }
   __syncthreads();
-  for (int i = threadIdx.x; i < NB; i += SORT_THREADS) hist[(u64)(tile - tile_base) * NB + i] = h[i];
+  for (int i = threadIdx.x; i < NB; i += SORT_THREADS) hist[(u64)tile * NB + i] = h[i];
 }
 #define RSS_WARPS 16
 template <int BITS>
-__global__ void __launch_bounds__(RSS_WARPS * 32) k_rs_scan(u32 *__restrict__ hist, const u32 *__restrict__ seg_tile0, u32 *__restrict__ digit_tot,
-                                                            u32 p_base = 0, u32 tile_base = 0) {
+__global__ void __launch_bounds__(RSS_WARPS * 32) k_rs_scan(u32 *__restrict__ hist, const u32 *__restrict__ seg_tile0, u32 *__restrict__ digit_tot) {
   constexpr int NB = 1 << BITS;
   __shared__ u32 part[RSS_WARPS][32];
-  const u32 p = blockIdx.x + p_base, d = blockIdx.y * 32 + lane_id();
+  const u32 p = blockIdx.x, d = blockIdx.y * 32 + lane_id();
   const int w = warp_id();
-  const u32 t0 = seg_tile0[p] - tile_base, t1 = seg_tile0[p + 1] - tile_base, nt = t1 - t0;
+  const u32 t0 = seg_tile0[p], t1 = seg_tile0[p + 1], nt = t1 - t0;
   const u32 per = (nt + RSS_WARPS - 1) / RSS_WARPS;
   const u32 a = t0 + (u32)w * per < t1 ? t0 + (u32)w * per : t1, b = a + per < t1 ? a + per : t1;
   u32 sum = 0;
@@ -220,13 +220,13 @@
 __global__ void __launch_bounds__(SORT_THREADS, 3) k_rs_scatter(const u64 *__restrict__ keys_in, u64 *__restrict__ keys_out,
                                                              const u32 *__restrict__ seg_cnt, const u32 *__restrict__ seg_tile0,
                                                              const u32 *__restrict__ tile_blk, int shift, const u32 *__restrict__ hist,
-                                                             const u32 *__restrict__ digit_tot, const u32 *__restrict__ seg_base, u32 tile_base = 0) {
+                                                             const u32 *__restrict__ digit_tot, const u32 *__restrict__ seg_base) {
   constexpr int NB = 1 << BITS;
   __shared__ u16 wcnt[SORT_THREADS / 32][NB];
   __shared__ u32 base[NB];
-  u32 tile = blockIdx.x + tile_base, p = tile_blk[tile];
+  u32 tile = blockIdx.x, p = tile_blk[tile];
   u32 cnt = seg_cnt[p], l0 = (tile - seg_tile0[p]) * SORT_TILE;
-  u64 gp = seg_base ? (u64)seg_base[p] : (u64)(seg_tile0[p] - tile_base) * SORT_TILE, g0 = gp + l0;
+  u64 gp = seg_base ? (u64)seg_base[p] : (u64)seg_tile0[p] * SORT_TILE, g0 = gp + l0;
   int lane = lane_id(), w = warp_id();
   for (int i = threadIdx.x; i < (SORT_THREADS / 32) * NB / 2; i += SORT_THREADS) reinterpret_cast<u32 *>(&wcnt[0][0])[i] = 0;
   {
@@ -234,7 +234,7 @@
     __shared__ u32 ws[33];
     u32 tot_d = threadIdx.x < NB ? digit_tot[(u64)p * NB + threadIdx.x] : 0u, tot;
     u32 ex = block_excl_sum<u32>(tot_d, tot, ws);
-    if (threadIdx.x < NB) base[threadIdx.x] = ex + hist[(u64)(tile - tile_base) * NB + threadIdx.x];
+    if (threadIdx.x < NB) base[threadIdx.x] = ex + hist[(u64)tile * NB + threadIdx.x];
   }
   __syncthreads();
   u64 key[SORT_E];
@@ -273,6 +273,100 @@
       keys_out[dst] = key[e];
     }
   }
+}
+
+#define R0_CAP 4096
+#define R0_ITEM_OTHER (1ull << 63)
+#define R0_PLAN_THREADS 128
+__global__ void __launch_bounds__(R0_PLAN_THREADS) k_r0_plan(const u32 *__restrict__ digit_tot, const u32 *__restrict__ seg_tile0,
+                                                             const u32 *__restrict__ seg_base, u64 item_flag, u64 *__restrict__ items,
+                                                             u32 item_cap, u32 *__restrict__ counts, u32 *__restrict__ nxt_cnt,
+                                                             u32 *__restrict__ nxt_base, u32 nxt_cap) {
+  __shared__ u32 c[512], it_lo[512], it_n[512], bg_lo[512], bg_n[512];
+  __shared__ u32 sh_ni, sh_nb, sh_i0, sh_b0;
+  const u32 p = blockIdx.x;
+  const u32 base = seg_base ? seg_base[p] : seg_tile0[p] * SORT_TILE;
+  for (int d = threadIdx.x; d < 512; d += R0_PLAN_THREADS) c[d] = digit_tot[(u64)p * 512 + d];
+  __syncthreads();
+  if (threadIdx.x == 0) {
+    u32 ni = 0, nbig = 0, pos = 0, st = 0, cur = 0;
+    for (int d = 0; d < 512; d++) {
+      const u32 k = c[d];
+      if (cur && (k > R0_CAP || cur + k > R0_CAP)) { it_lo[ni] = st; it_n[ni] = cur; ni++; cur = 0; }
+      if (k > R0_CAP) { bg_lo[nbig] = pos; bg_n[nbig] = k; nbig++; }
+      else if (k) { if (!cur) st = pos; cur += k; }
+      pos += k;
+    }
+    if (cur) { it_lo[ni] = st; it_n[ni] = cur; ni++; }
+    sh_ni = ni; sh_nb = nbig;
+    sh_i0 = atomicAdd(&counts[0], ni);
+    sh_b0 = atomicAdd(&counts[1], nbig);
+  }
+  __syncthreads();
+  for (u32 i = threadIdx.x; i < sh_ni; i += R0_PLAN_THREADS)
+    if (sh_i0 + i < item_cap) items[sh_i0 + i] = item_flag | (u64)it_n[i] << 32 | (u64)(base + it_lo[i]);
+  for (u32 i = threadIdx.x; i < sh_nb; i += R0_PLAN_THREADS)
+    if (sh_b0 + i < nxt_cap) { nxt_cnt[sh_b0 + i] = bg_n[i]; nxt_base[sh_b0 + i] = base + bg_lo[i]; }
+}
+#define R0_SORT_THREADS 512
+#define R0_E 8
+#define R0_SMEM (8 * (R0_CAP + R0_CAP / R0_E))
+static_assert(R0_SORT_THREADS * R0_E == R0_CAP, "one key per thread element");
+__device__ __forceinline__ u32 r0_pad(u32 i) { return i + (i >> 3); }
+__device__ __forceinline__ void r0_cswap(u64 &a, u64 &b) {
+  const u64 lo = a < b ? a : b, hi = a < b ? b : a;
+  a = lo;
+  b = hi;
+}
+__global__ void __launch_bounds__(R0_SORT_THREADS, 3) k_r0_bucket_sort(const u64 *__restrict__ items, u64 *dst, const u64 *other) {
+  DYN_SMEM(u64, sk);
+  const u64 it = items[blockIdx.x];
+  const u32 lo = (u32)it, n = (u32)(it >> 32) & 0x7fffffffu;
+  const u64 *src = (it & R0_ITEM_OTHER) ? other : dst;
+  u32 P = R0_E;
+  while (P < n) P <<= 1;
+  const u32 o = threadIdx.x * R0_E;
+  const bool act = o < P;
+  for (u32 i = threadIdx.x; i < P; i += R0_SORT_THREADS) sk[r0_pad(i)] = i < n ? src[lo + i] : ~0ull;
+  __syncthreads();
+  u64 k[R0_E];
+  if (act) {
+#pragma unroll
+    for (int e = 0; e < R0_E; e++) k[e] = sk[r0_pad(o + e)];
+    r0_cswap(k[0], k[1]); r0_cswap(k[2], k[3]); r0_cswap(k[4], k[5]); r0_cswap(k[6], k[7]);
+    r0_cswap(k[0], k[2]); r0_cswap(k[1], k[3]); r0_cswap(k[4], k[6]); r0_cswap(k[5], k[7]);
+    r0_cswap(k[1], k[2]); r0_cswap(k[5], k[6]);
+    r0_cswap(k[0], k[4]); r0_cswap(k[1], k[5]); r0_cswap(k[2], k[6]); r0_cswap(k[3], k[7]);
+    r0_cswap(k[2], k[4]); r0_cswap(k[3], k[5]);
+    r0_cswap(k[1], k[2]); r0_cswap(k[3], k[4]); r0_cswap(k[5], k[6]);
+  }
+  for (u32 w = R0_E; w <= P; w <<= 1) {
+    __syncthreads();
+    if (act) {
+#pragma unroll
+      for (int e = 0; e < R0_E; e++) sk[r0_pad(o + e)] = k[e];
+    }
+    __syncthreads();
+    if (w == P) break;
+    if (act) {
+      const u32 b = o & ~(2 * w - 1), diag = o - b, bA = b, bB = b + w;
+      u32 i0 = diag > w ? diag - w : 0, i1 = diag < w ? diag : w;
+      while (i0 < i1) {
+        const u32 m = (i0 + i1) >> 1;
+        if (sk[r0_pad(bA + m)] <= sk[r0_pad(bB + diag - 1 - m)]) i0 = m + 1; else i1 = m;
+      }
+      u32 i = i0, j = diag - i0;
+      u64 a = i < w ? sk[r0_pad(bA + i)] : ~0ull, c = j < w ? sk[r0_pad(bB + j)] : ~0ull;
+#pragma unroll
+      for (int e = 0; e < R0_E; e++) {
+        const bool ta = i < w && (j >= w || a <= c);
+        k[e] = ta ? a : c;
+        if (ta) { i++; a = i < w ? sk[r0_pad(bA + i)] : ~0ull; }
+        else { j++; c = j < w ? sk[r0_pad(bB + j)] : ~0ull; }
+      }
+    }
+  }
+  for (u32 i = threadIdx.x; i < n; i += R0_SORT_THREADS) dst[lo + i] = sk[r0_pad(i)];
 }
 
 __device__ __forceinline__ void seg_load_flags(const u64 *__restrict__ keys, u64 g0, u32 l0, u32 cnt, int kshift, u64 k[SEG_E], u32 &flags, u32 &lbase) {
@@ -340,7 +434,7 @@
                                                       const u32 *__restrict__ seg_tile0, const u32 *__restrict__ tile_blk,
                                                       u32 *__restrict__ isa, i64 stride, u32 *__restrict__ act_idx, u32 *__restrict__ act_rank,
                                                       u64 *__restrict__ status, u32 *__restrict__ ticket, u32 *__restrict__ n_act_out, u32 ntiles,
-                                                      const u8 *__restrict__ T, u8 *__restrict__ L, BlockRec *__restrict__ recs, u32 tile_base) {
+                                                      const u8 *__restrict__ T, u8 *__restrict__ L, BlockRec *__restrict__ recs) {
   __shared__ u64 sk[SORT_TILE + 2];
   __shared__ int wlast[R0_THREADS / 32];
   __shared__ u32 wkeep[R0_THREADS / 32];
@@ -351,7 +445,7 @@
   __syncthreads();
   const u32 tile = sh_tile, p = tile_blk[tile];
   const u32 cnt = seg_cnt[p], l0 = (tile - seg_tile0[p]) * SORT_TILE;
-  const u64 gp = (u64)(seg_tile0[p] - tile_base) * SORT_TILE;
+  const u64 gp = (u64)seg_tile0[p] * SORT_TILE;
   const u32 m = cnt - l0 < SORT_TILE ? cnt - l0 : SORT_TILE;
   for (u32 i = threadIdx.x; i < m + 2; i += R0_THREADS) {
     i64 j = (i64)l0 - 1 + i;
diff --git a/compressjs_flattened_b200/csrc/bz2b200.cu b/compressjs_flattened_b200/csrc/bz2b200.cu
--- a/compressjs_flattened_b200/csrc/bz2b200.cu
+++ b/compressjs_flattened_b200/csrc/bz2b200.cu
@@ -3,7 +3,6 @@
 #include "rle1.cuh"
 #include "bwt.cuh"
 #include "refine.cuh"
-#include "rsort2.cuh"
 #include "mtf.cuh"
 #include "huff.cuh"
 #include "decode.cuh"
@@ -99,7 +98,7 @@
   DevBuf isa, keysA, keysB, valsB, actI0, actI1, actR0, actR1, lb_status, lbm, hist, digit_base;
   DevBuf seg_cnt, seg_tile0, tile_blk, tile_i0, tile_i1, totals;
   DevBuf Lcol, ranks, lastocc, A, freq, meta, W, bit_off, scrc, out, out_len, used_bits;
-  DevBuf rs_tiles, gbounds;
+  DevBuf r0_item, r0_seg, r0_cnt, gbounds;
   DevBuf key2, big_cnt, big_old, big_rank, big_tile0, big_tblk, totals2;
   DevBuf recs_cand, cand_first, out2, recs_all, blksort, r2_status, hfreq, hlens, hplen, hcodes, hsel, hcost, hgoff, hblk;
   DevBuf d_in, cand, ncand, dmeta, dsyms, dL, dtt, dwalk, dblk, dout, dmisc, dsel, doff, dperm, dmap;
@@ -113,10 +112,8 @@
   bool trace = false;
   int sms = 148;
   unsigned ibwt_s = 64;
-  u32 r0_tiles = 1u << 30;
   u32 key_slack = 2;
   u32 key_bits = 44;
-  bool rs2 = false;
   int parse_mode = 0;
   std::vector<cudaEvent_t> trace_ev, trace_pool;
   std::vector<const char *> trace_names;
@@ -146,7 +143,7 @@
                      &isa, &keysA, &keysB, &valsB, &actI0, &actI1, &actR0, &actR1, &lb_status, &lbm, &hist, &digit_base,
                      &seg_cnt, &seg_tile0, &tile_blk, &tile_i0, &tile_i1, &totals,
                      &Lcol, &ranks, &lastocc, &A, &freq, &meta, &W, &bit_off, &scrc, &out, &out_len, &used_bits,
-                     &rs_tiles, &gbounds, &key2, &big_cnt, &big_old, &big_rank, &big_tile0, &big_tblk, &totals2,
+                     &r0_item, &r0_seg, &r0_cnt, &gbounds, &key2, &big_cnt, &big_old, &big_rank, &big_tile0, &big_tblk, &totals2,
                      &recs_cand, &cand_first, &out2, &recs_all, &blksort, &r2_status, &hfreq, &hlens, &hplen, &hcodes, &hsel, &hcost, &hgoff, &hblk,
                      &d_in, &cand, &ncand, &dmeta, &dsyms, &dL, &dtt, &dwalk, &dblk, &dout, &dmisc, &dsel, &doff, &dperm, &dmap};
     for (DevBuf *b : all) pool.push_back(b);
@@ -414,12 +411,7 @@
     if ((rc = mark(c, 1))) return rc;
 
     size_t slots = 0;
-    std::vector<u32> tiles_of((size_t)nb), tile_first((size_t)nb);
-    for (int b = 0; b < nb; b++) {
-      tile_first[(size_t)b] = (u32)(slots / SORT_TILE);
-      tiles_of[(size_t)b] = (u32)(round_up(hrecs[(size_t)b].n, SORT_TILE) / SORT_TILE);
-      slots += (size_t)tiles_of[(size_t)b] * SORT_TILE;
-    }
+    for (int b = 0; b < nb; b++) slots += (size_t)round_up(hrecs[(size_t)b].n, SORT_TILE);
     const size_t tiles0 = slots / SORT_TILE;
     if ((u64)nb * (u64)BS >= (1ull << 31)) { c->err = "too many bytes for one call (block table * stride must stay below 2^31)"; return BZ2B200_E_ARG; }
     const size_t big_tiles = 5 * tiles0 + 16;
@@ -450,13 +442,11 @@
     CK(cudaMemsetAsync(c->blksort.p, 0, sizeof(BlkSort) * (size_t)nb, c->stream));
     LAUNCH(k_sym_used, dim3(32, (unsigned)nb), 256, 0, P<u8>(c->blk), BS, P<BlockRec>(c->recs), P<BlkSort>(c->blksort));
     LAUNCH(k_sym_tab, (unsigned)nb, 256, 0, P<BlkSort>(c->blksort), c->key_bits, c->key_slack);
-    ENS(c->rs_tiles, sizeof(RsTile) * (size_t)(Ta + 1));
-    if (Ta) LAUNCH(k_rs_tiles, (Ta + 255) / 256, 256, 0, seg_cnt, tile0, tblk, (u32)Ta, P<RsTile>(c->rs_tiles));
     u64 total_n = 0;
     for (auto &r : hrecs) total_n += r.n;
     c->dom_used = 0;
     auto timed_scatter = [&](bool bits9, unsigned grid, const u64 *ki, u64 *ko, const u32 *scnt, const u32 *st0, const u32 *stb, int shift,
-                             const u32 *sbase, u64 slots_now, u32 tile_base) -> int {
+                             const u32 *sbase, u64 slots_now) -> int {
       if (c->ev_ok) {
         if (c->dom_used + 2 > c->dom_ev.size()) {
           cudaEvent_t a, b2;
@@ -465,8 +455,8 @@
         }
         CK(cudaEventRecord(c->dom_ev[c->dom_used], c->stream));
       }
-      if (bits9) LAUNCH(k_rs_scatter<9>, grid, SORT_THREADS, 0, ki, ko, scnt, st0, stb, shift, P<u32>(c->hist), P<u32>(c->digit_base), sbase, tile_base);
-      else LAUNCH(k_rs_scatter<8>, grid, SORT_THREADS, 0, ki, ko, scnt, st0, stb, shift, P<u32>(c->hist), P<u32>(c->digit_base), sbase, tile_base);
+      if (bits9) LAUNCH(k_rs_scatter<9>, grid, SORT_THREADS, 0, ki, ko, scnt, st0, stb, shift, P<u32>(c->hist), P<u32>(c->digit_base), sbase);
+      else LAUNCH(k_rs_scatter<8>, grid, SORT_THREADS, 0, ki, ko, scnt, st0, stb, shift, P<u32>(c->hist), P<u32>(c->digit_base), sbase);
       if (c->ev_ok) { CK(cudaEventRecord(c->dom_ev[c->dom_used + 1], c->stream)); c->dom_used += 2; }
       c->st.dom_launches++;
       c->st.dom_bytes += 16ull * slots_now;
@@ -478,47 +468,55 @@
       c->st.sort_slots += (u64)Ta * SORT_TILE;
       CK(cudaMemsetAsync(lbm, 0, 16, c->stream));
       CK(cudaMemsetAsync(status, 0, 8 * (size_t)Ta, c->stream));
-      for (int b0 = 0; b0 < nb;) {
-        u32 gt = 0;
-        int b1 = b0;
-        u64 gn = 0;
-        while (b1 < nb && (b1 == b0 || gt + tiles_of[b1] <= c->r0_tiles)) { gt += tiles_of[b1]; gn += hrecs[(size_t)b1].n; b1++; }
-        const u32 tb = tile_first[b0];
-        const unsigned gb = (unsigned)(b1 - b0);
-        LAUNCH(k_keys_init, gt, SEG_THREADS, 0, P<u8>(c->blk), BS, P<BlockRec>(c->recs), tile0, tblk, P<BlkSort>(c->blksort), kA, P<u32>(c->hist), tb, c->key_bits);
-        u64 *ki = kA, *ko = kB;
-        const int npass = (int)(c->key_bits + 8) / 9;
-        for (int pass = 0; pass < npass; pass++) {
-          if (pass) LAUNCH(k_rs_hist<9>, gt, SORT_THREADS, 0, ki, seg_cnt, tile0, tblk, 20 + pass * 9, P<u32>(c->hist), (const u32 *)nullptr, tb);
-          if (c->rs2 && tb == 0 && gt == Ta) {
-#if RS2_SCAN1
-            LAUNCH(k_rs_scan<9>, dim3((unsigned)nb, 512 / 32), RSS_WARPS * 32, 0, P<u32>(c->hist), tile0, P<u32>(c->digit_base), 0u, 0u);
-#else
-            LAUNCH(k_rs_bases, (unsigned)nb, 512, 0, P<u32>(c->hist), tile0);
-#endif
-            if (c->ev_ok) {
-              if (c->dom_used + 2 > c->dom_ev.size()) {
-                cudaEvent_t a, b2;
-                CK(cudaEventCreate(&a)); CK(cudaEventCreate(&b2));
-                c->dom_ev.push_back(a); c->dom_ev.push_back(b2);
-              }
-              CK(cudaEventRecord(c->dom_ev[c->dom_used], c->stream));
-            }
-            const unsigned g2 = gt < (unsigned)(2 * c->sms) ? gt : (unsigned)(2 * c->sms);
-            LAUNCH(k_rs_scatter2, g2, RS2_THREADS, sizeof(Rs2Smem), ki, ko, P<u32>(c->hist), P<RsTile>(c->rs_tiles), gt, 20 + pass * 9, P<u32>(c->digit_base));
-            if (c->ev_ok) { CK(cudaEventRecord(c->dom_ev[c->dom_used + 1], c->stream)); c->dom_used += 2; }
-            c->st.dom_launches++;
-            c->st.dom_bytes += 16ull * gn;
-          } else {
-            LAUNCH(k_rs_scan<9>, dim3(gb, 512 / 32), RSS_WARPS * 32, 0, P<u32>(c->hist), tile0, P<u32>(c->digit_base), (u32)b0, tb);
-            if ((rc = timed_scatter(true, gt, ki, ko, seg_cnt, tile0, tblk, 20 + pass * 9, nullptr, gn, tb))) return rc;
-          }
-          u64 *tk = ki; ki = ko; ko = tk;
+      const u32 item_cap = (u32)(10 * (slots / R0_CAP) + 2 * (size_t)nb + 16);
+      ENS(c->r0_item, 8 * (size_t)item_cap);
+      ENS(c->r0_seg, 4 * 4 * (size_t)big_cap);
+      ENS(c->r0_cnt, 16);
+      u32 *r0c = P<u32>(c->r0_cnt), *segl = P<u32>(c->r0_seg);
+      CK(cudaMemsetAsync(r0c, 0, 16, c->stream));
+      const int nlev = (int)(c->key_bits + 8) / 9;
+      u64 *const out_of[2] = {kB, kA};
+      u64 *const fin = out_of[(nlev - 1) & 1], *const other = fin == kA ? kB : kA;
+      int top = 20 + (int)c->key_bits;
+      LAUNCH(k_keys_init, Ta, SEG_THREADS, 0, P<u8>(c->blk), BS, P<BlockRec>(c->recs), tile0, tblk, P<BlkSort>(c->blksort), kA, P<u32>(c->hist),
+             (u32)(top - 9), c->key_bits);
+      const u32 *scnt = seg_cnt, *st0 = tile0, *stb = tblk, *sbase = nullptr;
+      u32 nseg = (u32)nb, ntl = Ta, n_items = 0;
+      u64 nkeys = total_n;
+      u64 *ki = kA;
+      for (int lev = 0;; lev++) {
+        const int bits = top - 20 < 9 ? top - 20 : 9, shift = top - bits;
+        u64 *ko = out_of[lev & 1];
+        if (bits == 9) {
+          if (lev) LAUNCH(k_rs_hist<9>, ntl, SORT_THREADS, 0, ki, scnt, st0, stb, shift, P<u32>(c->hist), sbase);
+          LAUNCH(k_rs_scan<9>, dim3(nseg, 512 / 32), RSS_WARPS * 32, 0, P<u32>(c->hist), st0, P<u32>(c->digit_base));
+        } else {
+          LAUNCH(k_rs_hist<8>, ntl, SORT_THREADS, 0, ki, scnt, st0, stb, shift, P<u32>(c->hist), sbase);
+          LAUNCH(k_rs_scan<8>, dim3(nseg, 256 / 32), RSS_WARPS * 32, 0, P<u32>(c->hist), st0, P<u32>(c->digit_base));
         }
-        LAUNCH(k_rank0, gt, R0_THREADS, 0, ki, seg_cnt, tile0, tblk, P<u32>(c->isa), BS, actI[0], actR[0], status, lbm, lbm + 1, (u32)Ta, P<u8>(c->blk),
-               P<u8>(c->Lcol), P<BlockRec>(c->recs), tb);
-        b0 = b1;
+        if ((rc = timed_scatter(bits == 9, ntl, ki, ko, scnt, st0, stb, shift, sbase, nkeys))) return rc;
+        top = shift;
+        if (top == 20) break;
+        u32 *ncnt = segl + (lev & 1) * 2 * big_cap, *nbase = ncnt + big_cap;
+        CK(cudaMemsetAsync(r0c + 1, 0, 4, c->stream));
+        LAUNCH(k_r0_plan, nseg, R0_PLAN_THREADS, 0, P<u32>(c->digit_base), st0, sbase, ko == fin ? 0ull : R0_ITEM_OTHER, P<u64>(c->r0_item), item_cap, r0c,
+               ncnt, nbase, big_cap);
+        LAUNCH(k_tilemap, 1, 1024, 0, ncnt, 0, P<u32>(c->big_tile0), P<u32>(c->big_tblk), P<u64>(c->totals2), r0c + 1);
+        u32 cn[4] = {0, 0, 0, 0};
+        u64 t2[2] = {0, 0};
+        RC(rb_add(c, cn, r0c, sizeof cn));
+        RC(rb_add(c, t2, c->totals2.p, sizeof t2));
+        RC(rb_sync(c));
+        if (cn[0] > item_cap || cn[1] > big_cap) { c->err = "internal: round-0 plan overflow"; return BZ2B200_E_CUDA; }
+        n_items = cn[0];
+        if (!cn[1]) break;
+        nseg = cn[1]; ntl = (u32)t2[0]; nkeys = t2[1];
+        scnt = ncnt; sbase = nbase; st0 = P<u32>(c->big_tile0); stb = P<u32>(c->big_tblk);
+        ki = ko;
       }
+      if (n_items) LAUNCH(k_r0_bucket_sort, n_items, R0_SORT_THREADS, R0_SMEM, P<u64>(c->r0_item), fin, other);
+      LAUNCH(k_rank0, Ta, R0_THREADS, 0, fin, seg_cnt, tile0, tblk, P<u32>(c->isa), BS, actI[0], actR[0], status, lbm, lbm + 1, (u32)Ta, P<u8>(c->blk),
+             P<u8>(c->Lcol), P<BlockRec>(c->recs));
       RC(rb_add(c, hv, lbm, sizeof hv));
       RC(rb_sync(c));
     }
@@ -554,7 +552,7 @@
         for (int pass = 0; pass < 3; pass++) {
           LAUNCH(k_rs_hist<8>, Tb, SORT_THREADS, 0, ki, bcnt, bt0, btb, 32 + pass * 8, P<u32>(c->hist), bbase);
           LAUNCH(k_rs_scan<8>, dim3(n_big, 256 / 32), RSS_WARPS * 32, 0, P<u32>(c->hist), bt0, P<u32>(c->digit_base));
-          if ((rc = timed_scatter(false, Tb, ki, ko, bcnt, bt0, btb, 32 + pass * 8, bbase, t2[1], 0u))) return rc;
+          if ((rc = timed_scatter(false, Tb, ki, ko, bcnt, bt0, btb, 32 + pass * 8, bbase, t2[1]))) return rc;
           u64 *tk = ki; ki = ko; ko = tk;
         }
         LAUNCH(k_sub_heads, Tb, SEG_THREADS, 0, ki, bcnt, bt0, btb, P<int>(c->tile_i0), bbase, 32);
@@ -806,7 +804,6 @@
 #ifndef BZ_SIM
   cudaError_t e;
   if ((e = cudaFuncSetAttribute(k_sort_groups, cudaFuncAttributeMaxDynamicSharedMemorySize, (int)sizeof(RfSmem))) != cudaSuccess) return e;
-  if ((e = cudaFuncSetAttribute(k_rs_scatter2, cudaFuncAttributeMaxDynamicSharedMemorySize, (int)sizeof(Rs2Smem))) != cudaSuccess) return e;
   if ((e = cudaFuncSetAttribute(k_mtf_ranks, cudaFuncAttributeMaxDynamicSharedMemorySize, (int)(MTR_WARPS * sizeof(MtrSmem)))) != cudaSuccess) return e;
   if ((e = cudaFuncSetAttribute(k_huf_init, cudaFuncAttributeMaxDynamicSharedMemorySize, (int)sizeof(HufBuildSmem))) != cudaSuccess) return e;
   if ((e = cudaFuncSetAttribute(k_huf_build, cudaFuncAttributeMaxDynamicSharedMemorySize, (int)sizeof(HufBuildSmem))) != cudaSuccess) return e;
@@ -829,8 +826,6 @@
   { const char *t = getenv("BZ2B200_PARSE"); c->parse_mode = t ? atoi(t) : 0; }
   { const char *t = getenv("BZ2B200_KEY_SLACK"); if (t && *t >= '0' && *t <= '3') c->key_slack = (u32)(*t - '0'); }
   { const char *t = getenv("BZ2B200_KEY_BITS"); int v = t ? atoi(t) : 0; if (v == 36 || v == 44 || v == 27) c->key_bits = (u32)v; }
-  { const char *t = getenv("BZ2B200_RS2"); if (t && *t) c->rs2 = *t != '0'; }
-  { const char *t = getenv("BZ2B200_R0_TILES"); int v = t ? atoi(t) : 0; if (v > 0) c->r0_tiles = (u32)v; }
   { const char *t = getenv("BZ2B200_IBWT_S"); int v = t ? atoi(t) : 0; if (v == 64 || v == 128 || v == 256 || v == 512 || v == 1024) c->ibwt_s = (unsigned)v; }
   { int v = 0; if (cudaDeviceGetAttribute(&v, cudaDevAttrMultiProcessorCount, device) == cudaSuccess && v > 0) c->sms = v; }
   for (auto &e : c->ev) if (cudaEventCreate(&e) != cudaSuccess) c->ev_ok = false;
diff --git a/compressjs_flattened_b200/csrc/rsort2.cuh b/compressjs_flattened_b200/csrc/rsort2.cuh
--- a/compressjs_flattened_b200/csrc/rsort2.cuh
+++ /dev/null
@@ -1,254 +0,0 @@
-#pragma once
-#include "common.cuh"
-#include "bwt.cuh"
-
-struct RsTile {
-  u32 p;
-  u32 m;
-  u32 g0;
-  u32 gp;
-};
-__global__ void k_rs_tiles(const u32 *__restrict__ seg_cnt, const u32 *__restrict__ seg_tile0, const u32 *__restrict__ tile_blk, u32 ntiles,
-                           RsTile *__restrict__ info) {
-  u32 t = blockIdx.x * blockDim.x + threadIdx.x;
-  if (t >= ntiles) return;
-  u32 p = tile_blk[t], l0 = (t - seg_tile0[p]) * SORT_TILE, cnt = seg_cnt[p];
-  RsTile r;
-  r.p = p; r.m = cnt - l0 < SORT_TILE ? cnt - l0 : SORT_TILE; r.g0 = t * SORT_TILE; r.gp = seg_tile0[p] * SORT_TILE;
-  info[t] = r;
-}
-
-__global__ void __launch_bounds__(512) k_rs_bases(u32 *__restrict__ hist, const u32 *__restrict__ seg_tile0) {
-  __shared__ u32 ws[33];
-  const u32 p = blockIdx.x, d = threadIdx.x;
-  const u32 t0 = seg_tile0[p], t1 = seg_tile0[p + 1];
-  u32 sum = 0;
-  for (u32 t = t0; t < t1; t++) sum += hist[(u64)t * 512 + d];
-  u32 tot;
-  u32 acc = block_excl_sum<u32>(sum, tot, ws);
-  for (u32 t = t0; t < t1; t++) {
-    const u32 v = hist[(u64)t * 512 + d];
-    hist[(u64)t * 512 + d] = acc;
-    acc += v;
-  }
-}
-
-#ifndef RS2_BALLOT
-#define RS2_BALLOT 0
-#endif
-#ifndef RS2_PACK
-#define RS2_PACK 1
-#endif
-#ifndef RS2_SCAN1
-#define RS2_SCAN1 1
-#endif
-#ifndef RS2_DIRECT
-#define RS2_DIRECT 0
-#endif
-#define RS2_THREADS 512
-#define RS2_WARPS (RS2_THREADS / 32)
-struct Rs2Smem {
-  u64 keys[2][SORT_TILE];
-  u32 gbase[2][512];
-#if RS2_SCAN1
-  u32 dtot[2][512];
-#endif
-#if RS2_PACK
-  u32 wcnt[RS2_WARPS / 2][512];
-#else
-  u32 wcnt[RS2_WARPS][512];
-#endif
-  u32 lpos[512];
-  u32 delta[512];
-  u32 ws[34];
-  u64 ws64[34];
-  RsTile info[2];
-  u64 mbar[2];
-};
-
-#ifndef BZ_SIM
-__device__ __forceinline__ u32 smem_u32(const void *p) { return (u32)__cvta_generic_to_shared(p); }
-__device__ __forceinline__ void mbar_init(u64 *bar, u32 count) { asm volatile("mbarrier.init.shared::cta.b64 [%0], %1;" ::"r"(smem_u32(bar)), "r"(count)); }
-__device__ __forceinline__ void mbar_expect_tx(u64 *bar, u32 bytes) {
-  asm volatile("mbarrier.arrive.expect_tx.shared::cta.b64 _, [%0], %1;" ::"r"(smem_u32(bar)), "r"(bytes) : "memory");
-}
-__device__ __forceinline__ void tma_load_1d(void *dst, const void *src, u32 bytes, u64 *bar) {
-  asm volatile("cp.async.bulk.shared::cluster.global.mbarrier::complete_tx::bytes [%0], [%1], %2, [%3];" ::"r"(smem_u32(dst)), "l"(src), "r"(bytes),
-               "r"(smem_u32(bar))
-               : "memory");
-}
-__device__ __forceinline__ void mbar_wait(u64 *bar, u32 parity) {
-  asm volatile(
-      "{\n"
-      ".reg .pred p;\n"
-      "RS2_WAIT:\n"
-      "mbarrier.try_wait.parity.shared::cta.b64 p, [%0], %1;\n"
-      "@p bra RS2_DONE;\n"
-      "bra RS2_WAIT;\n"
-      "RS2_DONE:\n"
-      "}\n" ::"r"(smem_u32(bar)),
-      "r"(parity)
-      : "memory");
-}
-#endif
-
-__device__ __forceinline__ void rs2_fetch(Rs2Smem &sm, int b, u32 tile, const u64 *__restrict__ keys_in, const u32 *__restrict__ hist,
-                                          const RsTile *__restrict__ tinfo, const u32 *__restrict__ digit_tot) {
-  const RsTile ti = tinfo[tile];
-  sm.info[b] = ti;
-  const u32 kbytes = ((ti.m * 8u) + 15u) & ~15u;
-#ifndef BZ_SIM
-  asm volatile("fence.proxy.async.shared::cta;" ::: "memory");
-  mbar_expect_tx(&sm.mbar[b], kbytes + 2048u * (1 + RS2_SCAN1));
-  tma_load_1d(sm.keys[b], keys_in + ti.g0, kbytes, &sm.mbar[b]);
-  tma_load_1d(sm.gbase[b], hist + (u64)tile * 512, 2048u, &sm.mbar[b]);
-#if RS2_SCAN1
-  tma_load_1d(sm.dtot[b], digit_tot + (u64)ti.p * 512, 2048u, &sm.mbar[b]);
-#endif
-#else
-  for (u32 i = 0; i < kbytes / 8; i++) sm.keys[b][i] = keys_in[ti.g0 + i];
-  for (u32 i = 0; i < 512; i++) sm.gbase[b][i] = hist[(u64)tile * 512 + i];
-#if RS2_SCAN1
-  for (u32 i = 0; i < 512; i++) sm.dtot[b][i] = digit_tot[(u64)ti.p * 512 + i];
-#endif
-#endif
-  (void)digit_tot;
-}
-
-__global__ void __launch_bounds__(RS2_THREADS, 2) k_rs_scatter2(const u64 *__restrict__ keys_in, u64 *__restrict__ keys_out, const u32 *__restrict__ hist,
-                                                                const RsTile *__restrict__ tinfo, u32 ntiles, int shift,
-                                                                const u32 *__restrict__ digit_tot) {
-  DYN_SMEM(Rs2Smem, smp);
-  Rs2Smem &sm = *smp;
-  const int lane = lane_id(), w = warp_id();
-  const u32 lt = (1u << lane) - 1;
-  if (threadIdx.x == 0) {
-#ifndef BZ_SIM
-    mbar_init(&sm.mbar[0], 1);
-    mbar_init(&sm.mbar[1], 1);
-    asm volatile("fence.mbarrier_init.release.cluster;" ::: "memory");
-#endif
-  }
-  __syncthreads();
-  u32 tile = blockIdx.x;
-  if (threadIdx.x == 0 && tile < ntiles) rs2_fetch(sm, 0, tile, keys_in, hist, tinfo, digit_tot);
-  for (u32 it = 0; tile < ntiles; it++, tile += gridDim.x) {
-    const int b = (int)(it & 1);
-    if (threadIdx.x == 0 && tile + gridDim.x < ntiles) rs2_fetch(sm, b ^ 1, tile + gridDim.x, keys_in, hist, tinfo, digit_tot);
-#ifndef BZ_SIM
-    mbar_wait(&sm.mbar[b], (it >> 1) & 1u);
-#else
-    __syncthreads();
-#endif
-    const u32 m = sm.info[b].m, gp = sm.info[b].gp;
-    u64 key[SORT_E];
-    u32 rk[SORT_E];
-#pragma unroll
-    for (int e = 0; e < SORT_E; e++) {
-      const u32 o = (u32)w * (32 * SORT_E) + e * 32 + lane;
-      key[e] = o < m ? sm.keys[b][o] : 0;
-    }
-#if RS2_PACK
-    for (int i = threadIdx.x; i < RS2_WARPS / 2 * 512; i += RS2_THREADS) (&sm.wcnt[0][0])[i] = 0;
-#else
-    for (int i = threadIdx.x; i < RS2_WARPS * 512; i += RS2_THREADS) (&sm.wcnt[0][0])[i] = 0;
-#endif
-    u32 dg[SORT_E], peers[SORT_E];
-#pragma unroll
-    for (int e = 0; e < SORT_E; e++) {
-      const u32 o = (u32)w * (32 * SORT_E) + e * 32 + lane;
-      dg[e] = o < m ? ((u32)(key[e] >> shift) & 511u) : 512u;
-#if RS2_BALLOT
-      u32 pm = __ballot_sync(FULL_MASK, o < m);
-      if (!(o < m)) pm = ~pm;
-#pragma unroll
-      for (int bit = 0; bit < 9; bit++) {
-        const bool one = (dg[e] >> bit) & 1u;
-        const u32 bal = __ballot_sync(FULL_MASK, one);
-        pm &= one ? bal : ~bal;
-      }
-      peers[e] = pm;
-#else
-      peers[e] = __match_any_sync(FULL_MASK, dg[e]);
-#endif
-    }
-    __syncthreads();
-#pragma unroll
-    for (int e = 0; e < SORT_E; e++) {
-      const int leader = __ffs((int)peers[e]) - 1;
-      u32 old = 0;
-#if RS2_PACK
-      if (lane == leader && dg[e] < 512u) old = (atomicAdd(&sm.wcnt[w >> 1][dg[e]], (u32)__popc(peers[e]) << (16 * (w & 1))) >> (16 * (w & 1))) & 0xffffu;
-#else
-      if (lane == leader && dg[e] < 512u) old = atomicAdd(&sm.wcnt[w][dg[e]], (u32)__popc(peers[e]));
-#endif
-      old = __shfl_sync(FULL_MASK, old, leader);
-      rk[e] = old + __popc(peers[e] & lt);
-    }
-    __syncthreads();
-    {
-      const u32 d = threadIdx.x;
-      u32 acc = 0;
-#if RS2_PACK
-      u32 cw[RS2_WARPS / 2];
-#pragma unroll
-      for (int q = 0; q < RS2_WARPS / 2; q++) {
-        const u32 v = sm.wcnt[q][d], lo = v & 0xffffu, hi = v >> 16;
-        cw[q] = acc | ((acc + lo) << 16);
-        acc += lo + hi;
-      }
-#if RS2_SCAN1
-      u64 tot64;
-      const u64 ex = block_excl_sum<u64>(((u64)sm.dtot[b][d] << 32) | acc, tot64, reinterpret_cast<u64 *>(sm.ws64));
-      const u32 lp = (u32)ex, dbase = (u32)(ex >> 32);
-#else
-      u32 tot;
-      const u32 lp = block_excl_sum<u32>(acc, tot, sm.ws);
-      const u32 dbase = 0;
-#endif
-#pragma unroll
-      for (int q = 0; q < RS2_WARPS / 2; q++) sm.wcnt[q][d] = cw[q] + lp * 0x10001u;
-#else
-      u32 cw[RS2_WARPS];
-#pragma unroll
-      for (int ww = 0; ww < RS2_WARPS; ww++) { cw[ww] = acc; acc += sm.wcnt[ww][d]; }
-      u32 tot;
-      const u32 lp = block_excl_sum<u32>(acc, tot, sm.ws);
-      const u32 dbase = 0;
-#pragma unroll
-      for (int ww = 0; ww < RS2_WARPS; ww++) sm.wcnt[ww][d] = lp + cw[ww];
-#endif
-      sm.lpos[d] = lp;
-      sm.delta[d] = dbase + sm.gbase[b][d] - lp;
-    }
-    __syncthreads();
-#if RS2_DIRECT
-#pragma unroll
-    for (int e = 0; e < SORT_E; e++)
-      if (dg[e] < 512u) {
-#if RS2_PACK
-        const u32 slot = ((sm.wcnt[w >> 1][dg[e]] >> (16 * (w & 1))) & 0xffffu) + rk[e];
-#else
-        const u32 slot = sm.wcnt[w][dg[e]] + rk[e];
-#endif
-        keys_out[(u64)gp + sm.delta[dg[e]] + slot] = key[e];
-      }
-#else
-#pragma unroll
-    for (int e = 0; e < SORT_E; e++)
-      if (dg[e] < 512u) {
-#if RS2_PACK
-        sm.keys[b][((sm.wcnt[w >> 1][dg[e]] >> (16 * (w & 1))) & 0xffffu) + rk[e]] = key[e];
-#else
-        sm.keys[b][sm.wcnt[w][dg[e]] + rk[e]] = key[e];
-#endif
-      }
-    __syncthreads();
-    for (u32 i = threadIdx.x; i < m; i += RS2_THREADS) {
-      const u64 k = sm.keys[b][i];
-      keys_out[(u64)gp + sm.delta[(u32)(k >> shift) & 511u] + i] = k;
-    }
-#endif
-    __syncthreads();
-  }
-}
```

Result: faster. 7528 (median of 6 runs) (+1.1%).
